# sinamalakouti/CDDMSL

Measured on AMD Instinct MI355X. Metric: images/sec (train step) VOC+Clipart RN50-C4, higher is better.
Workload: dtype bf16

## Files before the change

### __graft_entry__.py

```python
import glob
import os
import subprocess
import sys

ROOT = os.path.dirname(os.path.abspath(__file__))
CSRC = os.path.join(ROOT, "cddmsl_amd", "csrc")
LIB = os.path.join(ROOT, "cddmsl_amd", "libcddmsl_hip.so")
SIDE_LIBS = {"rpn_sparse.hip": os.path.join(ROOT, "cddmsl_amd", "libcddmsl_rpn_sparse.so")}
OBJDIR = os.path.join(ROOT, "build", "obj")
HIPCC = os.environ.get("HIPCC", "/opt/rocm/bin/hipcc")
HIPFLAGS = ["--offload-arch=gfx950", "-O3", "-fPIC", "-std=c++17", "-Wno-unused-result", "-ffp-contract=off"]


def _newer(src, dst, extra=()):
    if not os.path.exists(dst):
        return True
    t = os.path.getmtime(dst)
    return any(os.path.getmtime(s) > t for s in (src, *extra))


def build(verbose=False):
    os.makedirs(OBJDIR, exist_ok=True)
    headers = glob.glob(os.path.join(CSRC, "*.h")) + glob.glob(os.path.join(ROOT, "include", "*.h"))
    srcs = sorted(glob.glob(os.path.join(CSRC, "*.hip")))
    objs = []
    procs = []
    for s in srcs:
        o = os.path.join(OBJDIR, os.path.basename(s)[:-4] + ".o")
        objs.append(o)
        if _newer(s, o, headers):
            cmd = [HIPCC, *HIPFLAGS, "-I", os.path.join(ROOT, "include"), "-c", s, "-o", o]
            if verbose:
                print(" ".join(cmd))
            procs.append((s, subprocess.Popen(cmd)))
    for s, p in procs:
        if p.wait() != 0:
            raise RuntimeError(f"hipcc failed on {s}")
    side = {os.path.join(OBJDIR, name[:-4] + ".o"): lib for name, lib in SIDE_LIBS.items()}
    for lib, members in [(LIB, [o for o in objs if o not in side])] + [(lib, [o]) for o, lib in side.items()]:
        if not os.path.exists(lib) or any(os.path.getmtime(o) > os.path.getmtime(lib) for o in members):
            subprocess.check_call([HIPCC, "--offload-arch=gfx950", "-shared", "-fPIC", *members, "-o", lib])
    omk = os.path.join(ROOT, "oracle", "Makefile")
    if os.path.exists(omk):
        subprocess.check_call(["make", "-s", "-C", os.path.join(ROOT, "oracle")])
    if ROOT not in sys.path:
        sys.path.insert(0, ROOT)
    import cddmsl_amd
    from cddmsl_amd import _lib

    _lib.lib()
    _lib.lib_rpn_sparse()


def smoke():
    if ROOT not in sys.path:
        sys.path.insert(0, ROOT)
    import torch
    from cddmsl_amd import _lib, synthetic
    from cddmsl_amd.config import get_cfg
    from cddmsl_amd.engine import SimpleTrainer
    from cddmsl_amd.modeling import TransformerMapper, build_model
    from cddmsl_amd.solver import build_optimizer
    _lib.lib()
    assert torch.cuda.is_available(), "smoke() needs the MI355X"
    cfg = get_cfg()
    cfg.merge_from_file(os.path.join(ROOT, "configs", "VOC-Experiments", "faster_rcnn_CLIP_R_50_C4.yaml"))
    cfg.merge_from_list(["MODEL.COMPUTE_DTYPE", "f32", "MODEL.ROI_HEADS.BATCH_SIZE_PER_IMAGE", 16, "MODEL.RPN.PRE_NMS_TOPK_TRAIN", 300,
                         "MODEL.RPN.POST_NMS_TOPK_TRAIN", 100, "MODEL.DEVICE", "cuda:0"])
    sd, msd = synthetic.make_state_dict(0), synthetic.make_mapper_state_dict(1)
    model = build_model(cfg)
    model.load_state_dict(sd, strict=False)
    mapper = TransformerMapper(compute_dtype=model.compute_dtype)
    mapper.load_state_dict(msd)
    mapper.to(model.device)
    g = torch.Generator().manual_seed(3)
    model.proposal_generator.sample_generator = model.roi_heads.sample_generator = model.region_generator = g
    batch = synthetic.make_batch(1, 128, 160, num_gt=2)
    tr = SimpleTrainer(model, iter([batch]), build_optimizer(cfg, model), cfg, clipcap_model=mapper, metrics_period=0)
    tr.iter = 20000
    losses = tr.run_step()
    got = {k: float(v.detach()) for k, v in losses.items()}

    from oracle import model as om
    ocfg = om.Cfg(roi_batch_per_image=16, rpn_pre_nms_topk=300, rpn_post_nms_topk=100)
    torch.set_num_threads(min(16, os.cpu_count() or 8))
    with torch.no_grad():
        ref = om.run_step_losses(sd, msd, ocfg, batch, 20000, torch.Generator().manual_seed(3))
    for k, v in ref.items():
        assert abs(got[k] - float(v)) <= 1e-3 * abs(float(v)) + 1e-6, (k, got[k], float(v))
    print("smoke ok:", got)


if __name__ == "__main__":
    build(verbose=True)
    print("built", LIB)
```

### cddmsl_amd/_lib.py

```python
import ctypes
import os
import re

import torch

_HERE = os.path.dirname(os.path.abspath(__file__))
LIB_PATH = os.path.join(_HERE, "libcddmsl_hip.so")
HEADER_PATH = os.path.join(os.path.dirname(_HERE), "include", "cddmsl_hip.h")
RPN_SPARSE_LIB_PATH = os.path.join(_HERE, "libcddmsl_rpn_sparse.so")
RPN_SPARSE_HEADER_PATH = os.path.join(os.path.dirname(_HERE), "include", "cddmsl_rpn_sparse.h")

_lib = None
_lib_rpn_sparse = None


class HipLibraryError(RuntimeError):
    pass


_BY_VALUE = {"int": ctypes.c_int, "long": ctypes.c_long, "float": ctypes.c_float}


def _statements(header_text):
    text = re.sub(r"/\*.*?\*/", " ", header_text, flags=re.S)
    text = re.sub(r"^\s*#.*$", " ", text, flags=re.M)
    text = re.sub(r'extern\s+"C"\s*\{|^\s*\}\s*$', " ", text, flags=re.M)
    return [" ".join(s.split()) for s in text.split(";") if s.strip()]


def header_signatures(header_text):
    sigs = {}
    for st in _statements(header_text):
        if "(" not in st:
            continue
        m = re.fullmatch(r"(.*?)\b(cddmsl_\w+) ?\((.*)\)", st)
        if m is None:
            raise HipLibraryError(f"include/cddmsl_hip.h: cannot parse the declaration `{st}`")
        ret, name, params = m.group(1).strip(), m.group(2), m.group(3).strip()
        if ret != "int":
            raise HipLibraryError(f"include/cddmsl_hip.h: {name} returns `{ret}`; every entry point returns int")
        argtypes = []
        for p in ([] if params == "void" else params.split(",")):
            if "*" in p:
                argtypes.append(ctypes.c_void_p)
                continue
            words = [w for w in p.split() if w != "const"]
            if len(words) != 2 or words[0] not in _BY_VALUE:
                raise HipLibraryError(f"include/cddmsl_hip.h: {name}: parameter `{p.strip()}` is neither a pointer nor a "
                                      "by-value int / long / float")
            argtypes.append(_BY_VALUE[words[0]])
        sigs[name] = argtypes
    return sigs


def header_struct(header_text, name):
    m = re.search(r"typedef struct %s \{(.*?)\} %s;" % (name, name), re.sub(r"/\*.*?\*/", " ", header_text, flags=re.S), flags=re.S)
    if m is None:
        raise HipLibraryError(f"include/cddmsl_hip.h: no struct {name}")
    fields = []
    for st in (s.split() for s in m.group(1).split(";") if s.strip()):
        if st[0] not in ("int", "long"):
            raise HipLibraryError(f"include/cddmsl_hip.h: struct {name}: unknown member type in `{' '.join(st)}`")
        fields += [(w.strip(","), _BY_VALUE[st[0]]) for w in st[1:]]
    return fields


def _load(lib_path, header_path):
    if not os.path.exists(lib_path):
        raise HipLibraryError(
            f"{lib_path} is missing: run `python -c 'import __graft_entry__ as g; g.build()'` "
            "(hipcc --offload-arch=gfx950).  cddmsl_amd has no fallback path."
        )
    L = ctypes.CDLL(lib_path)
    with open(header_path) as f:
        sigs = header_signatures(f.read())
    for name, argtypes in sigs.items():
        fn = getattr(L, name, None)
        if fn is None:
            raise HipLibraryError(f"{lib_path} is stale: it does not export {name}, which include/{os.path.basename(header_path)} declares; rebuild it")
        fn.restype, fn.argtypes = ctypes.c_int, argtypes
    return L


def lib():
    global _lib
    if _lib is None:
        _lib = _load(LIB_PATH, HEADER_PATH)
    return _lib


def lib_rpn_sparse():
    global _lib_rpn_sparse
    if _lib_rpn_sparse is None:
        _lib_rpn_sparse = _load(RPN_SPARSE_LIB_PATH, RPN_SPARSE_HEADER_PATH)
    return _lib_rpn_sparse


def stream_ptr():
    return ctypes.c_void_p(torch._C._cuda_getCurrentRawStream(torch.cuda.current_device()))


def to_device_async(cpu_tensor, device):
    if torch.device(device).type == "cpu":
        return cpu_tensor
    if cpu_tensor.numel() == 0:
        return torch.empty(cpu_tensor.shape, dtype=cpu_tensor.dtype, device=device)
    return cpu_tensor.pin_memory().to(device, non_blocking=True)


def ptr(t):
    if t is None:
        return ctypes.c_void_p(0)
    return ctypes.c_void_p(t.data_ptr())


def check(status, what):
    if status != 0:
        raise HipLibraryError(f"{what} failed with status {status}")


def require_cuda(*tensors):
    for t in tensors:
        if t is not None and not t.is_cuda:
            raise HipLibraryError(
                "cddmsl_amd ops run only on the MI355X HIP path; got a CPU tensor "
                "(the CPU restatement lives in oracle/ and is test infrastructure only)"
            )


class Readback:

    def __init__(self, t):
        if t.is_cuda:
            self.host = torch.empty(t.shape, dtype=t.dtype, pin_memory=True)
            self.host.copy_(t, non_blocking=True)
            self.ev = torch.cuda.Event()
            self.ev.record()
        else:
            self.host, self.ev = t, None

    def get(self):
        if self.ev is not None:
            self.ev.synchronize()
        return self.host
```

### cddmsl_amd/csrc/conv_wgrad.hip

```cpp
#include "gemm_common.h"

namespace {

template <typename T> struct TrFrag;
template <> struct TrFrag<__bf16> {
  __device__ static __forceinline__ u32x4 read(const u32x4* base, int mrow0, int col0, int lane) {
    int g = lane >> 4, li = lane & 15, q = li >> 2, pp = li & 3;
    int hh = g >> 1;
    int col = col0 + 16 * (g & 1) + 4 * pp;
    const char* b = (const char*)base;
    const char* a0 = b + (long)(mrow0 + 8 * hh + q) * (WROW * 16) + col * 2;
    const char* a1 = a0 + 4 * (WROW * 16);
    i16x4 v0 = __builtin_amdgcn_ds_read_tr16_b64_v4i16((__attribute__((address_space(3))) i16x4*)a0);
    i16x4 v1 = __builtin_amdgcn_ds_read_tr16_b64_v4i16((__attribute__((address_space(3))) i16x4*)a1);
    u32x2 p0 = __builtin_bit_cast(u32x2, v0), p1 = __builtin_bit_cast(u32x2, v1);
    u32x4 r = {p0[0], p0[1], p1[0], p1[1]};
    return r;
  }
  static constexpr int MSTEP = 16;
};
template <> struct TrFrag<float> {
  __device__ static __forceinline__ u32x4 read(const u32x4* base, int mrow0, int col0, int lane) {
    int r = lane & 31, hh = lane >> 5;
    const char* b = (const char*)base;
// ... 83 lines not shown
    for (int ms = 0; ms < WM; ms += TrFrag<T>::MSTEP) {
      u32x4 fa[NT], fb[NT];
#pragma unroll
      for (int i = 0; i < NT; ++i) {
        fa[i] = TrFrag<T>::read(lds[0], ms, wn * WT + i * 32, lane);
        fb[i] = TrFrag<T>::read(lds[1], ms, wk * WT + i * 32, lane);
      }
#pragma unroll
      for (int a = 0; a < NT; ++a)
#pragma unroll
        for (int b = 0; b < NT; ++b) Mma<T>::step(acc[a][b], fa[a], fb[b]);
    }
    __syncthreads();
  }

  const int r = lane & 31, h = lane >> 5;
#pragma unroll
  for (int a = 0; a < NT; ++a)
#pragma unroll
    for (int b = 0; b < NT; ++b) {
      int k = k0 + wk * WT + b * 32 + r;
      if (k >= p.K) continue;
#pragma unroll
      for (int g = 0; g < 16; ++g) {
        int n = n0 + wn * WT + a * 32 + (g & 3) + 8 * (g >> 2) + 4 * h;
        if (n >= p.Cout) continue;
        float v = acc[a][b][g] * (p.scale ? p.scale[n] : 1.f);
        atomicAdd(p.dw + (long)n * p.K + k, v);
      }
    }
}


template <typename T> struct TrFragS;
template <> struct TrFragS<__bf16> {
  struct Off { int o0, o1; };
  __device__ static __forceinline__ Off prep(int col0, int lane) {
    int g = lane >> 4, li = lane & 15, q = li >> 2, pp = li & 3;
    int hh = g >> 1;
    int ch = ((col0 + 16 * (g & 1)) >> 3) + (pp >> 1);
    int r0 = 8 * hh + q, r1 = r0 + 4;
    Off o;
    o.o0 = r0 * 256 + 16 * (ch ^ fsw(r0)) + 8 * (pp & 1);
    o.o1 = r1 * 256 + 16 * (ch ^ fsw(r1)) + 8 * (pp & 1);
    return o;
  }
  __device__ static __forceinline__ u32x4 read(const u32x4* base, int ms, const Off& o) {
    const unsigned a = (unsigned)(size_t)(const __attribute__((address_space(3))) char*)((const char*)base) + ms * 256;
    u32x2 p0, p1;
    asm volatile("ds_read_b64_tr_b16 %0, %1" : "=v"(p0) : "v"(a + o.o0));
    asm volatile("ds_read_b64_tr_b16 %0, %1" : "=v"(p1) : "v"(a + o.o1));
    u32x4 r = {p0[0], p0[1], p1[0], p1[1]};
    return r;
  }
  static constexpr int MSTEP = 16;
};
template <> struct TrFragS<float> {
  struct Off { int o[4]; };
  __device__ static __forceinline__ Off prep(int col0, int lane) {
    int r = lane & 31, hh = lane >> 5;
    int byte = (col0 + r) * 4;
    Off o;
#pragma unroll
    for (int j = 0; j < 4; ++j) {
      int row = 4 * hh + j;
      o.o[j] = row * 256 + (byte & 15) + 16 * (byte >> 4);
    }
    return o;
  }
  __device__ static __forceinline__ u32x4 read(const u32x4* base, int ms, const Off& o) {
    const char* b = (const char*)base;
    u32x4 v;
#pragma unroll
    for (int j = 0; j < 4; ++j) {
      int off = o.o[j] + ms * 256;
      int row = off >> 8, ch = (off >> 4) & 15;
      v[j] = *(const unsigned int*)(b + (off & ~0xf0) + 16 * (ch ^ fsw(row)));
    }
    return v;
  }
  static constexpr int MSTEP = 8;
};

template <typename T>
__global__ __launch_bounds__(256, 2) void k_conv_wgrad_dma(WgradArgs p) {
  constexpr int ES = Mma<T>::ES;
  constexpr int COLS = 256 / ES;
  __shared__ __attribute__((aligned(16))) u32x4 lds[2][2][WM * 16];
  const int t = threadIdx.x, lane = t & 63, wv = t >> 6;
  p.x += (long)blockIdx.y * p.bx; p.dy += (long)blockIdx.y * p.bd;
  char* outp = (char*)p.dw + (long)blockIdx.y * p.bo;
  const int wvu = __builtin_amdgcn_readfirstlane(t >> 6);
  const int ntn = (p.Cout + COLS - 1) / COLS, ntk = (p.K + COLS - 1) / COLS;
  int bid = xcd_remap(blockIdx.x, gridDim.x);
  const int tile_k = bid % ntk; bid /= ntk;
  const int tile_n = bid % ntn; bid /= ntn;
  const int split = bid;
  const int n0 = tile_n * COLS, k0 = tile_k * COLS;
  const int mt0 = split * p.mtiles_per_split;
  const int total_mt = (p.M + WM - 1) / WM;
  const int mt1 = min(mt0 + p.mtiles_per_split, total_mt);

  const int cc = t & 15, rb = t >> 4;
  const int cl = cc ^ fsw(rb);
  const int kc = k0 * ES / 16 + cl;
  const bool vk = kc < p.Kc;
  const int pp = vk ? kc / p.cpp : 0, coff = vk ? kc - pp * p.cpp : 0;
  const int ky = pp / p.KW, kx = pp - ky * p.KW;
  const int nc = n0 * ES / 16 + cl;
  const bool vn = nc < p.ncc;
  const bool taps = !(p.KH == 1 && p.KW == 1);
  const char* zp = (const char*)g_zero_page;

  int m[4];
  const char* pd[4];
  const char* px[4];
#pragma unroll
  for (int i = 0; i < 4; ++i) {
    m[i] = mt0 * WM + rb + 16 * i;
    pd[i] = p.dy + ((long)m[i] * p.ldd) * ES + (long)nc * 16;
    px[i] = p.x + (((long)m[i] + (long)(ky - p.pad) * p.Wi + (kx - p.pad)) * p.xrs) * 16 + (long)coff * 16;
  }
  const long dstep = (long)WM * p.ldd * ES, xstep = (long)WM * p.xrs * 16;

  auto stage = [&](int buf) {
#pragma unroll
    for (int i = 0; i < 4; ++i) {
      bool vmm = m[i] < p.M;
      glds16((vmm && vn) ? pd[i] : zp, &lds[buf][0][(4 * wvu + 16 * i) * 16]);
    }
#pragma unroll
    for (int i = 0; i < 4; ++i) {
      bool ok = (m[i] < p.M) & vk;
      if (taps) {
        unsigned mm = min((unsigned)m[i], (unsigned)(p.M - 1));
        unsigned tq = fdiv(mm, p.dWo);
        unsigned ox = mm - tq * p.Wo;
        unsigned oy = tq - fdiv(tq, p.dHo) * p.Ho;
        ok = ok & ((unsigned)((int)oy - p.pad + ky) < (unsigned)p.Hi) & ((unsigned)((int)ox - p.pad + kx) < (unsigned)p.Wi);
      }
      glds16(ok ? px[i] : zp, &lds[buf][1][(4 * wvu + 16 * i) * 16]);
    }
#pragma unroll
    for (int i = 0; i < 4; ++i) { m[i] += WM; pd[i] += dstep; px[i] += xstep; }
  };

  constexpr int WT = COLS / 2;
  constexpr int NT = WT / 32;
  const int wn = wv >> 1, wk = wv & 1;
  f32x16 acc[NT][NT];
#pragma unroll
  for (int a = 0; a < NT; ++a)
#pragma unroll
    for (int b = 0; b < NT; ++b)
#pragma unroll
      for (int r = 0; r < 16; ++r) acc[a][b][r] = 0.f;

  typename TrFragS<T>::Off offa[NT], offb[NT];
#pragma unroll
  for (int i = 0; i < NT; ++i) {
    offa[i] = TrFragS<T>::prep(wn * WT + i * 32, lane);
    offb[i] = TrFragS<T>::prep(wk * WT + i * 32, lane);
  }

  if (mt0 < mt1) stage(0);
  for (int mt = mt0; mt < mt1; ++mt) {
    const int cur = (mt - mt0) & 1;
    if (mt + 1 < mt1) {
      stage(cur ^ 1);
      asm volatile("s_waitcnt vmcnt(8)" ::: "memory");
    } else {
      asm volatile("s_waitcnt vmcnt(0)" ::: "memory");
    }
    __builtin_amdgcn_s_barrier();
#pragma unroll
    for (int ms = 0; ms < WM; ms += TrFragS<T>::MSTEP) {
      u32x4 fa[NT], fb[NT];
#pragma unroll
      for (int i = 0; i < NT; ++i) {
        fa[i] = TrFragS<T>::read(lds[cur][0], ms, offa[i]);
        fb[i] = TrFragS<T>::read(lds[cur][1], ms, offb[i]);
      }
      asm volatile("s_waitcnt lgkmcnt(0)" ::: "memory");
      __builtin_amdgcn_sched_barrier(0);
#pragma unroll
      for (int a = 0; a < NT; ++a)
#pragma unroll
        for (int b = 0; b < NT; ++b) Mma<T>::step(acc[a][b], fa[a], fb[b]);
    }
    asm volatile("s_waitcnt lgkmcnt(0)" ::: "memory");
    __builtin_amdgcn_s_barrier();
  }

  const int r = lane & 31, h = lane >> 5;
  if (p.ws) {
    f32x4* dst = (f32x4*)p.ws + ((long)(split * ntn + tile_n) * ntk + tile_k) * (4 * NT * NT * 4 * 64) + (wv * NT * NT * 4) * 64 + lane;
#pragma unroll
    for (int a = 0; a < NT; ++a)
#pragma unroll
      for (int b = 0; b < NT; ++b)
#pragma unroll
        for (int g4 = 0; g4 < 4; ++g4) {
          const f32x4 v = {acc[a][b][4 * g4], acc[a][b][4 * g4 + 1], acc[a][b][4 * g4 + 2], acc[a][b][4 * g4 + 3]};
          dst[((a * NT + b) * 4 + g4) * 64] = v;
        }
    return;
  }
#pragma unroll
  for (int a = 0; a < NT; ++a)
#pragma unroll
    for (int b = 0; b < NT; ++b) {
      int k = k0 + wk * WT + b * 32 + r;
      if (k >= p.K) continue;
#pragma unroll
      for (int g = 0; g < 16; ++g) {
        int n = n0 + wn * WT + a * 32 + (g & 3) + 8 * (g >> 2) + 4 * h;
        if (n >= p.Cout) continue;
        float v = acc[a][b][g] * (p.scale ? p.scale[n] : 1.f);
        long o = (long)n * p.ldo + k;
        if (p.direct == 0) atomicAdd((float*)outp + o, v);
        else if (p.direct == 1) ((float*)outp)[o] = v;
        else Mma<T>::store(outp + o * ES, v);
      }
    }
}

template <typename T>
__global__ __launch_bounds__(256, 2) void k_gemm_tn_stream(WgradArgs p, int nbatch, int bpb) {
  constexpr int ES = Mma<T>::ES;
  constexpr int COLS = 256 / ES;
  __shared__ __attribute__((aligned(16))) u32x4 lds[2][2][WM * 16];
  const int t = threadIdx.x, lane = t & 63, wv = t >> 6;
  const int wvu = __builtin_amdgcn_readfirstlane(t >> 6);
  const int ntk = (p.K + COLS - 1) / COLS;
  const int tile_k = blockIdx.x % ntk, tile_n = blockIdx.x / ntk;
  const int n0 = tile_n * COLS, k0 = tile_k * COLS;
  const int b0 = blockIdx.y * bpb, nb = min(bpb, nbatch - b0);
  const int nmt = (p.M + WM - 1) / WM;
  const int nit = nb * nmt;

  const int cc = t & 15, rb = t >> 4;
  const int cl = cc ^ fsw(rb);
  const int kc = k0 * ES / 16 + cl, nc = n0 * ES / 16 + cl;
  const bool vk = kc < p.Kc, vn = nc < p.ncc;
  const char* zp = (const char*)g_zero_page;
  int sb = 0, smt = 0;
  auto stage = [&](int buf) {
    const char* db = p.dy + (long)(b0 + sb) * p.bd + (long)nc * 16;
    const char* xb = p.x + (long)(b0 + sb) * p.bx + (long)kc * 16;
#pragma unroll
    for (int i = 0; i < 4; ++i) {
      const int m = smt * WM + rb + 16 * i;
// ... 185 lines not shown
    const unsigned x0 = sbase + xoff[0], x1 = sbase + xoff[1];
    CDDMSL_TRS(fb[0], x0, x1, 0) CDDMSL_TRS(fb[1], x0, x1, 4096) CDDMSL_TRS(fb[2], x0, x1, 8192) CDDMSL_TRS(fb[3], x0, x1, 12288)
#pragma unroll
    for (int a = 0; a < NTN; ++a) {
      const unsigned a0 = sbase + aoff[a][0], a1 = sbase + aoff[a][1];
      CDDMSL_TRS(fa[a][0], a0, a1, 0) CDDMSL_TRS(fa[a][1], a0, a1, 2048) CDDMSL_TRS(fa[a][2], a0, a1, 4096) CDDMSL_TRS(fa[a][3], a0, a1, 6144)
    }
#undef CDDMSL_TRS
    if (NTN == 1) asm volatile("s_waitcnt lgkmcnt(0)" : "+v"(fb[0]), "+v"(fb[1]), "+v"(fb[2]), "+v"(fb[3]), "+v"(fa[0][0]), "+v"(fa[0][1]),
                               "+v"(fa[0][2]), "+v"(fa[0][3]) :: "memory");
    else asm volatile("s_waitcnt lgkmcnt(0)" : "+v"(fb[0]), "+v"(fb[1]), "+v"(fb[2]), "+v"(fb[3]), "+v"(fa[0][0]), "+v"(fa[0][1]), "+v"(fa[0][2]),
                      "+v"(fa[0][3]), "+v"(fa[NTN - 1][0]), "+v"(fa[NTN - 1][1]), "+v"(fa[NTN - 1][2]), "+v"(fa[NTN - 1][3]) :: "memory");
    __builtin_amdgcn_sched_barrier(0);
#pragma unroll
    for (int ms = 0; ms < 4; ++ms)
#pragma unroll
      for (int a = 0; a < NTN; ++a) Mma<__bf16>::step(acc[a], fa[a][ms], fb[ms]);
    __builtin_amdgcn_s_barrier();
    char* outp = (char*)p.dw + (long)(b0 + it) * p.bo;
    const int k = k0 + wvu * 32 + r;
    if (MODE == 3) {
      if (kind == 2) asm volatile("s_waitcnt vmcnt(6)" : "+v"(g0v), "+v"(mbv) :: "memory");
      else asm volatile("s_waitcnt vmcnt(0)" : "+v"(g0v), "+v"(mbv) :: "memory");
      const unsigned a00 = __builtin_bit_cast(unsigned, acc[0][0]);
      const float t0 = __builtin_bit_cast(float, __builtin_amdgcn_permlane32_swap(a00, a00, false, false)[0]) + g0v;
      const float base = t0 * (1.0f / (float)(P > 0 ? P : 1));
      const unsigned mlo = mbv[0], mhi = mbv[1];
#pragma unroll
      for (int a = 0; a < NTN; ++a)
#pragma unroll
        for (int g = 0; g < 16; ++g) {
          const int n0 = a * 32 + (g & 3) + 8 * (g >> 2);
          const bool exists = a * 4 + (g >> 2) < NG;
          const bool lo_ok = n0 >= 1 && n0 <= P, hi_ok = n0 + 4 >= 1 && n0 + 4 <= P;
          if (exists) {
            const int n = n0 + 4 * h;
            const float v = acc[a][g];
            gacc[a][g] += (n == 0) ? t0 : v;
            if (lo_ok || hi_ok) {
              if (h ? hi_ok : lo_ok) {
                const unsigned word = (n - 1) < 32 ? mlo : mhi;
                const bool keep = (word >> ((n - 1) & 31)) & 1u;
                Mma<__bf16>::store(outp + ((long)(n - 1) * p.ldo + k) * 2, keep ? v + base : 0.f);
              }
            }
          }
          acc[a][g] = 0.f;
        }
      return;
    }
#pragma unroll
    for (int a = 0; a < NTN; ++a)
#pragma unroll
      for (int g = 0; g < 16; ++g) {
        if (a * 4 + (g >> 2) < NG) {
          const int n = a * 32 + (g & 3) + 8 * (g >> 2) + 4 * h;
          const float v = acc[a][g];
          const long o = (long)n * p.ldo + k;
          if (MODE == 0) atomicAdd((float*)outp + o, v);
          else if (MODE == 1) ((float*)outp)[o] = v;
          else Mma<__bf16>::store(outp + o * 2, v);
        }
        acc[a][g] = 0.f;
      }
  };
  {
    int it = 0;
    for (; it + 2 < nit; ++it) item(it, std::integral_constant<int, 2>{});
    if (it + 1 < nit) { item(it, std::integral_constant<int, 1>{}); ++it; }
    if (it < nit) item(it, std::integral_constant<int, 0>{});
  }
  if (MODE == 3 && p.gpos) {
    const int k = k0 + wvu * 32 + r;
#pragma unroll
    for (int a = 0; a < NTN; ++a)
#pragma unroll
      for (int g = 0; g < 16; ++g) {
        const int n = a * 32 + (g & 3) + 8 * (g >> 2) + 4 * h;
        if (a * 4 + (g >> 2) < NG && n <= P) atomicAdd(p.gpos + (long)n * p.K + k, gacc[a][g]);
      }
  }
}

__global__ __launch_bounds__(512) void k_wgrad256(WgradArgs p) {
  __shared__ __attribute__((aligned(16))) u32x4 lds[2 * 2 * 2 * 64 * 16];
  const int t = threadIdx.x, lane = t & 63;
#ifdef CDDMSL_TILE_STAMPS
  const unsigned long long ts_entry = __builtin_amdgcn_s_memrealtime();
  unsigned long long ts_loop = ts_entry;
#endif
  p.x += (long)blockIdx.y * p.bx; p.dy += (long)blockIdx.y * p.bd;
  char* outp = (char*)p.dw + (long)blockIdx.y * p.bo;
  const int wvu = __builtin_amdgcn_readfirstlane(t >> 6);
  const int wn = wvu >> 2, wk = wvu & 3;
  const int ntn = p.Cout >> 8, ntk = p.K >> 8;
  int bid = xcd_remap(blockIdx.x, gridDim.x);
  const int tile_k = bid % ntk; bid /= ntk;
  const int tile_n = bid % ntn; bid /= ntn;
  const int n0 = tile_n * 256, k0 = tile_k * 256;
  const int mt0 = bid * p.mtiles_per_split;
  const int nmt = min(p.mtiles_per_split, (p.M + WM - 1) / WM - mt0);
  const bool taps = !(p.KH == 1 && p.KW == 1);

  const int rb = t >> 4, cl = (t & 15) ^ fsw(rb);
  const int gd = (cl >> 3) * 16 + (cl & 7);
  const int gx = (cl >> 2) * 8 + (cl & 3);
  const int kc = (k0 >> 3) + gx;
  const int pp = kc / p.cpp, coff = kc - pp * p.cpp;
  const int ky = pp / p.KW, kx = pp - ky * p.KW;
  unsigned vd[2], vx[2];
#pragma unroll
  for (int i = 0; i < 2; ++i) {
    vd[i] = (unsigned)((i * 32 + rb) * p.ldd * 2 + gd * 16);
    vx[i] = (unsigned)((((i * 32 + rb) + ky * p.Wi + kx) * p.xrs + coff) * 16);
  }
  const __amdgpu_buffer_rsrc_t rd = __builtin_amdgcn_make_buffer_rsrc((void*)(p.dy + ((long)mt0 * WM * p.ldd + n0) * 2), 0, 0x80000000u, 0x00020000);
  const __amdgpu_buffer_rsrc_t rx = __builtin_amdgcn_make_buffer_rsrc((void*)(p.x + ((long)mt0 * WM - p.pad * p.Wi - p.pad) * p.xrs * 16), 0, 0x80000000u, 0x00020000);
  const unsigned dstep = (unsigned)(WM * p.ldd * 2), xstep = (unsigned)(WM * p.xrs * 16);
  const int mrow = mt0 * WM + rb;

  char* const L = (char*)lds;
  auto stageD = [&](auto H, int buf, int T) {
    constexpr int h = decltype(H)::value;
    char* dst = L + (buf << 16) + (h << 14) + wvu * 1024;
#pragma unroll
    for (int i = 0; i < 2; ++i) {
      const unsigned inv = (mrow + T * WM + i * 32 < p.M) ? 0u : 0x80000000u;
      __builtin_amdgcn_raw_ptr_buffer_load_lds(rd, (__attribute__((address_space(3))) void*)(dst + i * 8192 - h * 128), 16,
                                               (int)(vd[i] | inv), (int)(T * dstep), h * 128, 0);
    }
  };
  unsigned xinv[2];
  auto validX = [&](int T) {
#pragma unroll
    for (int i = 0; i < 2; ++i) {
      const int m = mrow + T * WM + i * 32;
      bool ok = m < p.M;
      if (taps) {
        const unsigned mm = min((unsigned)m, (unsigned)(p.M - 1));
        const unsigned tq = fdiv(mm, p.dWo);
        const unsigned ox = mm - tq * p.Wo;
        const unsigned oy = tq - fdiv(tq, p.dHo) * p.Ho;
        ok = ok & ((unsigned)((int)oy - p.pad + ky) < (unsigned)p.Hi) & ((unsigned)((int)ox - p.pad + kx) < (unsigned)p.Wi);
      }
      xinv[i] = ok ? 0u : 0x80000000u;
    }
  };
  auto stageX = [&](auto J, int buf, int T) {
    constexpr int j = decltype(J)::value;
    char* dst = L + (buf << 16) + (1 << 15) + (j << 14) + wvu * 1024;
#pragma unroll
    for (int i = 0; i < 2; ++i)
      __builtin_amdgcn_raw_ptr_buffer_load_lds(rx, (__attribute__((address_space(3))) void*)(dst + i * 8192 - j * 64), 16,
                                               (int)(vx[i] | xinv[i]), (int)(T * xstep), j * 64, 0);
  };
  using I0 = std::integral_constant<int, 0>;
  using I1 = std::integral_constant<int, 1>;

  f32x16 acc[4][2];
#pragma unroll
  for (int a = 0; a < 4; ++a)
#pragma unroll
    for (int b = 0; b < 2; ++b)
#pragma unroll
      for (int r = 0; r < 16; ++r) acc[a][b][r] = 0.f;

  const unsigned lbase = (unsigned)(size_t)(__attribute__((address_space(3))) char*)L;
  unsigned adA[2][2], adB[2];
  {
#pragma unroll
    for (int a = 0; a < 2; ++a) {
      const TrFragS<__bf16>::Off o = TrFragS<__bf16>::prep(wn * 64 + a * 32, lane);
      adA[a][0] = lbase + o.o0; adA[a][1] = lbase + o.o1;
    }
    const TrFragS<__bf16>::Off o = TrFragS<__bf16>::prep(wk * 32, lane);
    adB[0] = lbase + (1u << 15) + o.o0; adB[1] = lbase + (1u << 15) + o.o1;
  }
  u32x4 fa0[2][4], fa1[2][4], fb0[4], fb1[4];
#define CDDMSL_TR2(DST, A0, A1, IMM)                                                             \
  { u32x2 q0_, q1_;                                                                              \
    asm volatile("ds_read_b64_tr_b16 %0, %1 offset:%2" : "=v"(q0_) : "v"(A0), "i"(IMM));         \
    asm volatile("ds_read_b64_tr_b16 %0, %1 offset:%2" : "=v"(q1_) : "v"(A1), "i"(IMM));         \
    DST = u32x4{q0_[0], q0_[1], q1_[0], q1_[1]}; }
#define CDDMSL_READ_A(HALF, FA)                                                                  \
  _Pragma("unroll") for (int a = 0; a < 2; ++a) {                                                \
    CDDMSL_TR2(FA[a][0], adA[a][0], adA[a][1], ((HALF) << 14) + 0 * 4096)                        \
    CDDMSL_TR2(FA[a][1], adA[a][0], adA[a][1], ((HALF) << 14) + 1 * 4096)                        \
    CDDMSL_TR2(FA[a][2], adA[a][0], adA[a][1], ((HALF) << 14) + 2 * 4096)                        \
    CDDMSL_TR2(FA[a][3], adA[a][0], adA[a][1], ((HALF) << 14) + 3 * 4096) }
#define CDDMSL_READ_B(HALF, FB)                                                                  \
  CDDMSL_TR2(FB[0], adB[0], adB[1], ((HALF) << 14) + 0 * 4096)                                   \
  CDDMSL_TR2(FB[1], adB[0], adB[1], ((HALF) << 14) + 1 * 4096)                                   \
  CDDMSL_TR2(FB[2], adB[0], adB[1], ((HALF) << 14) + 2 * 4096)                                   \
  CDDMSL_TR2(FB[3], adB[0], adB[1], ((HALF) << 14) + 3 * 4096)
#define CDDMSL_FLIP_A() { adA[0][0] ^= 1u << 16; adA[0][1] ^= 1u << 16; adA[1][0] ^= 1u << 16; adA[1][1] ^= 1u << 16; }
#define CDDMSL_FLIP_B() { adB[0] ^= 1u << 16; adB[1] ^= 1u << 16; }
#define CDDMSL_MMA_QUAD(I, J, FA, FB)                                               \
  _Pragma("unroll") for (int ms = 0; ms < 4; ++ms) {                                \
    Mma<__bf16>::step(acc[2 * (I)][J], FA[0][ms], FB[ms]);                          \
    Mma<__bf16>::step(acc[2 * (I) + 1][J], FA[1][ms], FB[ms]);                      \
  }
#define CDDMSL_WAIT4(F) asm volatile("s_waitcnt lgkmcnt(0)" : "+v"(F[0]), "+v"(F[1]), "+v"(F[2]), "+v"(F[3]) :: "memory");
#define CDDMSL_WAIT8(F) asm volatile("s_waitcnt lgkmcnt(0)" : "+v"(F[0][0]), "+v"(F[0][1]), "+v"(F[0][2]), "+v"(F[0][3]), \
                                     "+v"(F[1][0]), "+v"(F[1][1]), "+v"(F[1][2]), "+v"(F[1][3]) :: "memory");
#define CDDMSL_PHASE_SYNC_IN(WAIT)                                                  \
  __builtin_amdgcn_sched_barrier(0);                                                \
  __builtin_amdgcn_s_barrier();                                                     \
  WAIT                                                                              \
  __builtin_amdgcn_sched_barrier(0);                                                \
  __builtin_amdgcn_s_setprio(1);
#define CDDMSL_PHASE_SYNC_OUT(I, J)                                                 \
  asm volatile("" : "+v"(acc[2 * (I)][J]), "+v"(acc[2 * (I) + 1][J]));              \
  __builtin_amdgcn_s_setprio(0);                                                    \
  __builtin_amdgcn_sched_barrier(0);                                                \
  __builtin_amdgcn_s_barrier();                                                     \
  __builtin_amdgcn_sched_barrier(0);

  if (nmt > 0) {
    validX(0);
    stageD(I0{}, 0, 0); stageD(I1{}, 0, 0); stageX(I0{}, 0, 0); stageX(I1{}, 0, 0);
    if (nmt > 1) {
      validX(1);
      stageD(I0{}, 1, 1); stageX(I0{}, 1, 1); stageX(I1{}, 1, 1);
      asm volatile("s_waitcnt vmcnt(6)" ::: "memory");
    } else {
      asm volatile("s_waitcnt vmcnt(0)" ::: "memory");
    }
    __builtin_amdgcn_s_barrier();
    __builtin_amdgcn_sched_barrier(0);
    CDDMSL_READ_A(0, fa0)
    CDDMSL_WAIT8(fa0)
    if (wn == 1) __builtin_amdgcn_s_barrier();
    __builtin_amdgcn_sched_barrier(0);
// ... 201 lines not shown
      const unsigned a0 = adA[0] + ro, a1 = adA[1] + ro, b0 = adB[0] + ro, b1 = adB[1] + ro;
      CDDMSL_TR8x4(fa[0], a0)
      mma(IS{}, I2{}, I0{});
      CDDMSL_TR8x4(fa[1], a1)
      mma(IS{}, I2{}, I1{});
      CDDMSL_TR8x4(fb[N][0], b0)
      mma(IS{}, I3{}, I0{});
      CDDMSL_TR8x4(fb[N][1], b1)
      mma(IS{}, I3{}, I1{});
    }
  };
  if (nmt > 0) {
    stage(0);
    if (nmt > 1) stage(1);
    if (nmt > 2) stage(2);
    if (nmt > 2) asm volatile("s_waitcnt vmcnt(8)" ::: "memory");
    else if (nmt > 1) asm volatile("s_waitcnt vmcnt(4)" ::: "memory");
    else asm volatile("s_waitcnt vmcnt(0)" ::: "memory");
    __builtin_amdgcn_sched_barrier(0);
    __builtin_amdgcn_s_barrier();
    __builtin_amdgcn_sched_barrier(0);
    CDDMSL_TR8x4(fa[0], adA[0]) CDDMSL_TR8x4(fa[1], adA[1]) CDDMSL_TR8x4(fb[0][0], adB[0]) CDDMSL_TR8x4(fb[0][1], adB[1])
    for (int kt = 0; kt < nmt; kt += 2) {
      body(kt, I0{});
      body(kt + 1, I1{});
    }
  }
#undef CDDMSL_TR8x4
#undef CDDMSL_F8_WAIT_TOP
#undef CDDMSL_F8_WAIT_MID
#undef CDDMSL_TR8

  const int r = lane & 31, h = lane >> 5;
  if (p.ws) {
    store_frags((f32x4*)p.ws + ((long)(bid * ntn + tile_n) * ntk + tile_k) * (8 * 32 * 64) + (wvu * 32) * 64 + lane, acc);
  } else
#pragma unroll
  for (int a = 0; a < 4; ++a)
#pragma unroll
    for (int b = 0; b < 2; ++b) {
      const int k = k0 + wk * 64 + b * 32 + r;
#pragma unroll
      for (int g = 0; g < 16; ++g) {
        const int n = n0 + wn * 128 + a * 32 + (g & 3) + 8 * (g >> 2) + 4 * h;
        atomicAdd(p.dw + (long)n * p.ldo + k, acc[a][b][g] * (p.scale ? p.scale[n] : 1.f));
      }
    }
}

}

template <int WAVES, int FR>
__global__ __launch_bounds__(256) void k_wgrad_reduce(const f32x4* ws, float* dw, const float* scale, int ntn, int ntk, int splits, int Cout, int K, int ldo) {
  constexpr int SLOTS = WAVES * FR * 64;
  constexpr int TN = WAVES == 8 ? 256 : 128;
  const int tile = blockIdx.x / (SLOTS / 256), q = (blockIdx.x % (SLOTS / 256)) * 256 + threadIdx.x;
  const int tile_k = tile % ntk, tile_n = tile / ntk;
  const long ntiles = (long)ntn * ntk;
  const f32x4* src = ws + (long)tile * SLOTS + q;
  f32x4 sum = {0.f, 0.f, 0.f, 0.f};
  int s = 0;
  for (; s + 4 <= splits; s += 4) {
    const f32x4 a = src[(s + 0) * ntiles * SLOTS], b = src[(s + 1) * ntiles * SLOTS], c = src[(s + 2) * ntiles * SLOTS], d = src[(s + 3) * ntiles * SLOTS];
    sum += (a + b) + (c + d);
  }
  for (; s < splits; ++s) sum += src[s * ntiles * SLOTS];
  const int wv = q / (FR * 64), j = (q / 64) % FR, lane = q & 63, r = lane & 31, h = lane >> 5, g4 = j & 3;
  int a, b, wn, wk;
  if (WAVES == 8) { a = j >> 3; b = (j >> 2) & 1; wn = wv >> 2; wk = wv & 3; }
  else { a = j >> 3; b = (j >> 2) & 1; wn = wv >> 1; wk = wv & 1; }
  const int n = tile_n * TN + wn * (WAVES == 8 ? 128 : 64) + a * 32 + 8 * g4 + 4 * h;
  const int k = tile_k * TN + wk * 64 + b * 32 + r;
  if (k >= K) return;
#pragma unroll
  for (int e = 0; e < 4; ++e)
    if (n + e < Cout) dw[(long)(n + e) * ldo + k] += sum[e] * (scale ? scale[n + e] : 1.f);
}

static bool use_workspace(long blocks, long tile_floats, void* ws, long ws_bytes) {
  if (env_int("CDDMSL_WGRAD_WS", 1) == 0) return false;
  return ws != nullptr && blocks * tile_floats * 4 <= ws_bytes;
}

template <int WAVES, int FR>
static void launch_wgrad_split(void (*kernel)(WgradArgs), WgradArgs& a, const Plan& p, hipStream_t st, void* wsp, long ws_bytes) {
  constexpr int TN = WAVES == 8 ? 256 : 128, SLOTS = WAVES * FR * 64;
  const int ntn = (a.Cout + TN - 1) / TN, ntk = (a.K + TN - 1) / TN;
  const bool ws = p.splits > 1 && use_workspace((long)p.gx, SLOTS * 4, wsp, ws_bytes);
  if (ws) a.ws = (float*)wsp;
  hipLaunchKernelGGL(kernel, dim3(p.gx), dim3(WAVES * 64), 0, st, a);
  if (ws) hipLaunchKernelGGL((k_wgrad_reduce<WAVES, FR>), dim3((unsigned)(ntn * ntk * (SLOTS / 256))), dim3(256), 0, st, (const f32x4*)wsp, a.dw, a.scale,
                             ntn, ntk, p.splits, a.Cout, a.K, a.ldo);
}

void launch_wgrad(WgradArgs& a, const Plan& p, Operand op, hipStream_t st, void* ws, long ws_bytes) {
  switch (p.kernel) {
    case 12: launch_wgrad_split<8, 32>(k_wgrad256_f8, a, p, st, ws, ws_bytes); break;
    case 6: launch_wgrad_split<8, 32>(k_wgrad256, a, p, st, ws, ws_bytes); break;
    case 5:
      if (op == OP_BF16) launch_wgrad_split<4, 16>(k_conv_wgrad_dma<__bf16>, a, p, st, ws, ws_bytes);
      else hipLaunchKernelGGL(k_conv_wgrad_dma<float>, dim3(p.gx), dim3(256), 0, st, a);
      break;
    default:
      if (op == OP_BF16) hipLaunchKernelGGL(k_conv_wgrad<__bf16>, dim3(p.gx), dim3(256), 0, st, a);
      else hipLaunchKernelGGL(k_conv_wgrad<float>, dim3(p.gx), dim3(256), 0, st, a);
  }
}

void launch_gemm_tn(const WgradArgs& p, Operand op, const Plan& pl, int batch, int mode, hipStream_t st) {
  const dim3 grid(pl.gx, pl.gy);
  if (pl.kernel == 9) {
#define CDDMSL_TNS(NG)                                                                                              \
  case NG:                                                                                                          \
    if (mode == 0) hipLaunchKernelGGL((k_gemm_tn_small<NG, 0>), grid, dim3(256), 0, st, p, batch, pl.bpb);      \
    else if (mode == 1) hipLaunchKernelGGL((k_gemm_tn_small<NG, 1>), grid, dim3(256), 0, st, p, batch, pl.bpb); \
    else hipLaunchKernelGGL((k_gemm_tn_small<NG, 2>), grid, dim3(256), 0, st, p, batch, pl.bpb);                \
    break;
    switch (p.Cout / 8) { CDDMSL_TNS(1) CDDMSL_TNS(2) CDDMSL_TNS(3) CDDMSL_TNS(4) CDDMSL_TNS(5) CDDMSL_TNS(6) CDDMSL_TNS(7) CDDMSL_TNS(8) }
#undef CDDMSL_TNS
  } else if (pl.kernel == 7) {
    if (op == OP_BF16) hipLaunchKernelGGL(k_gemm_tn_stream<__bf16>, grid, dim3(256), 0, st, p, batch, pl.bpb);
    else hipLaunchKernelGGL(k_gemm_tn_stream<float>, grid, dim3(256), 0, st, p, batch, pl.bpb);
  } else {
    if (op == OP_BF16) hipLaunchKernelGGL(k_conv_wgrad_dma<__bf16>, grid, dim3(256), 0, st, p);
    else hipLaunchKernelGGL(k_conv_wgrad_dma<float>, grid, dim3(256), 0, st, p);
  }
}

void launch_attnpool_dx(const WgradArgs& p, unsigned gx, unsigned gy, int nbatch, int bpb, hipStream_t st) {
  hipLaunchKernelGGL((k_gemm_tn_small<7, 3, 49>), dim3(gx, gy), dim3(256), 0, st, p, nbatch, bpb);
}
```

### cddmsl_amd/csrc/gemm_common.h

```cpp
#pragma once
#include "common.h"
#include <cstdlib>

namespace {

constexpr int BM = 128, BN = 128, KCH = 8;

struct FastDiv {
  unsigned mul, shr, d;
};
static inline FastDiv make_fastdiv(unsigned d) {
  FastDiv f;
  f.d = d;
  unsigned s = 0;
  while ((1ull << s) < d) ++s;
  f.shr = s;
  f.mul = (unsigned)(((1ull << 32) * ((1ull << s) - d)) / d + 1);
  return f;
}
__device__ __forceinline__ unsigned fdiv(unsigned n, const FastDiv& f) { return (__umulhi(n, f.mul) + n) >> f.shr; }

template <typename T> __device__ __forceinline__ float affine(float v, float sc, float bi) {
  return sizeof(T) <= 2 ? __builtin_fmaf(v, sc, bi) : v * sc + bi;
}
// ... 31 lines not shown
  FastDiv dWp = {}, dHp = {};
  int nt_out = 1;
#ifdef CDDMSL_TILE_STAMPS
  unsigned long long* tstamps = nullptr;
#endif
};

template <typename T> struct Mma;
template <> struct Mma<__bf16> {
  static constexpr int ES = 2;
  __device__ static __forceinline__ void step(f32x16& acc, const u32x4& a, const u32x4& b) {
    acc = __builtin_amdgcn_mfma_f32_32x32x16_bf16(__builtin_bit_cast(bf16x8, a), __builtin_bit_cast(bf16x8, b), acc, 0, 0, 0);
  }
  __device__ static __forceinline__ float load(const char* p) { return bf2f(*(const unsigned short*)p); }
  __device__ static __forceinline__ void store(char* p, float v) { *(unsigned short*)p = f2bf(v); }
};
template <> struct Mma<float> {
  static constexpr int ES = 4;
  __device__ static __forceinline__ void step(f32x16& acc, const u32x4& a, const u32x4& b) {
    const f32x4 fa = __builtin_bit_cast(f32x4, a), fb = __builtin_bit_cast(f32x4, b);
    acc = __builtin_amdgcn_mfma_f32_32x32x2f32(fa[0], fb[0], acc, 0, 0, 0);
    acc = __builtin_amdgcn_mfma_f32_32x32x2f32(fa[1], fb[1], acc, 0, 0, 0);
    acc = __builtin_amdgcn_mfma_f32_32x32x2f32(fa[2], fb[2], acc, 0, 0, 0);
    acc = __builtin_amdgcn_mfma_f32_32x32x2f32(fa[3], fb[3], acc, 0, 0, 0);
  }
  __device__ static __forceinline__ float load(const char* p) { return *(const float*)p; }
  __device__ static __forceinline__ void store(char* p, float v) { *(float*)p = v; }
};
typedef __attribute__((ext_vector_type(8))) int i32x8;

__device__ __forceinline__ int xcd_remap(int bid, int nblk) {
  const int q = nblk >> 3, rem = nblk & 7, x = bid & 7, j = bid >> 3;
  return (x < rem ? x * (q + 1) : rem * (q + 1) + (x - rem) * q) + j;
}

template <typename T> __device__ __forceinline__ u32x4 avg4(const u32x4& a, const u32x4& b, const u32x4& c, const u32x4& d);
template <> __device__ __forceinline__ u32x4 avg4<float>(const u32x4& a, const u32x4& b, const u32x4& c, const u32x4& d) {
  const f32x4 fa = __builtin_bit_cast(f32x4, a), fb = __builtin_bit_cast(f32x4, b);
  const f32x4 fc = __builtin_bit_cast(f32x4, c), fd = __builtin_bit_cast(f32x4, d);
  f32x4 r = ((fa + fb) + (fc + fd)) * 0.25f;
  return __builtin_bit_cast(u32x4, r);
}
template <> __device__ __forceinline__ u32x4 avg4<__bf16>(const u32x4& a, const u32x4& b, const u32x4& c, const u32x4& d) {
  u32x4 r;
#pragma unroll
  for (int j = 0; j < 4; ++j) {
    float lo = (bf2f(a[j] & 0xffff) + bf2f(b[j] & 0xffff)) + (bf2f(c[j] & 0xffff) + bf2f(d[j] & 0xffff));
    float hi = (bf2f(a[j] >> 16) + bf2f(b[j] >> 16)) + (bf2f(c[j] >> 16) + bf2f(d[j] >> 16));
    r[j] = pack2bf(lo * 0.25f, hi * 0.25f);
  }
  return r;
}

__device__ __attribute__((aligned(16))) unsigned int g_zero_page[4] = {0u, 0u, 0u, 0u};

__device__ __forceinline__ void glds16(const void* g, void* l) {
  __builtin_amdgcn_global_load_lds((const __attribute__((address_space(1))) void*)g,
                                   (__attribute__((address_space(3))) void*)l, 16, 0, 0);
}

struct WgradArgs {
  const char* x;
  const char* dy;
  float* dw;
  const float* scale;
  int Nimg, Hi, Wi, Cin, Ho, Wo, Cout, KH, KW, stride, pad, ldd, pool;
  int M, Kc, cpp, K, ncc;
  int mtiles_per_split;
  FastDiv dWo, dHo;
  int xrs;
  int ldo;
  int direct;
  long bx, bd, bo;
  const float* g0 = nullptr;
  const unsigned long long* mbits = nullptr;
  float* gpos = nullptr;
  float* ws = nullptr;
#ifdef CDDMSL_TILE_STAMPS
  unsigned long long* tstamps = nullptr;
#endif
};

constexpr int WM = 64;
constexpr int WROW = 16 + 4;

__device__ __forceinline__ int fsw(int row) { return ((row & 3) << 2) | ((row >> 2) & 3); }

__device__ __forceinline__ void store_frags(f32x4* dst, const f32x16 (&acc)[4][2]) {
#pragma unroll
  for (int a = 0; a < 4; ++a)
#pragma unroll
    for (int b = 0; b < 2; ++b)
#pragma unroll
      for (int g4 = 0; g4 < 4; ++g4) {
        const f32x4 v = {acc[a][b][4 * g4], acc[a][b][4 * g4 + 1], acc[a][b][4 * g4 + 2], acc[a][b][4 * g4 + 3]};
        dst[((a * 2 + b) * 4 + g4) * 64] = v;
      }
}

static long env_int(const char* name, long dflt, bool* set = nullptr) {
  const char* e = getenv(name);
  if (set) *set = e != nullptr;
  return e ? atol(e) : dflt;
}

enum Operand { OP_BF16 = 0, OP_F32 = 1, OP_FP8 = 2 };
static int elem_size(Operand op) { return op == OP_BF16 ? 2 : op == OP_F32 ? 4 : 1; }

struct Plan {
  int kernel;
  unsigned gx, gy;
  int splits;
  int mtiles_per_split;
  int bpb;
};

static int persistent_blocks_raw() {
  static int ncu = -1;
  if (ncu < 0) {
    int dev = 0, n = 0;
    if (hipGetDevice(&dev) != hipSuccess || hipDeviceGetAttribute(&n, hipDeviceAttributeMultiprocessorCount, dev) != hipSuccess) n = 0;
    ncu = (n / 8) * 8;
  }
  return ncu;
}

}

extern "C" {
__attribute__((visibility("hidden"))) void launch_fwd_tile128(const ConvArgs& a, const Plan& p, Operand op, hipStream_t st);
__attribute__((visibility("hidden"))) void launch_fwd_tile256(const ConvArgs& a, const Plan& p, Operand op, hipStream_t st, void* ws, long ws_bytes);
__attribute__((visibility("hidden"))) void launch_wgrad(WgradArgs& a, const Plan& p, Operand op, hipStream_t st, void* ws, long ws_bytes);
__attribute__((visibility("hidden"))) void launch_gemm_tn(const WgradArgs& p, Operand op, const Plan& pl, int batch, int mode, hipStream_t st);
__attribute__((visibility("hidden"))) void launch_attnpool_dx(const WgradArgs& p, unsigned gx, unsigned gy, int nbatch, int bpb, hipStream_t st);
__attribute__((visibility("hidden"))) bool record_kernel(int id);
}
```

### cddmsl_amd/csrc/gemm_conv.hip

```cpp
#include "gemm_common.h"

namespace {

template <typename T>
__device__ __forceinline__ void weight_prep_body(const float* w, const float* scale, char* wf, char* wd, int Cout, int KH, int KW, int Cin,
                                                 long first, long stride) {
  __shared__ float tile[32][33];
  const int taps = KH * KW, nit = (Cin + 31) / 32, nct = (Cout + 31) / 32;
  const long ntiles = (long)nct * taps * nit;
  const int tx = threadIdx.x & 31, ty = threadIdx.x >> 5;
  constexpr int ES = Mma<T>::ES;
  for (long tl = first; tl < ntiles; tl += stride) {
    const int it = (int)(tl % nit); const long q = tl / nit;
    const int tap = (int)(q % taps), ct = (int)(q / taps);
    const int ky = tap / KW, kx = tap % KW;
    __syncthreads();
#pragma unroll
    for (int r = 0; r < 4; ++r) {
      const int co = ct * 32 + ty + 8 * r, ci = it * 32 + tx;
      float v = 0.f;
      if (co < Cout && ci < Cin) {
        const long i = ((long)co * taps + tap) * Cin + ci;
        v = w[i];
        if (wf) Mma<T>::store(wf + i * ES, v);
        if (scale) v *= scale[co];
      }
      tile[ty + 8 * r][tx] = v;
    }
    __syncthreads();
    if (wd) {
#pragma unroll
      for (int r = 0; r < 4; ++r) {
        const int ci = it * 32 + ty + 8 * r, co = ct * 32 + tx;
        if (ci < Cin && co < Cout) {
          const long j = (((long)ci * KH + (KH - 1 - ky)) * KW + (KW - 1 - kx)) * Cout + co;
          Mma<T>::store(wd + j * ES, tile[tx][ty + 8 * r]);
        }
      }
    }
  }
}
template <typename T>
__global__ __launch_bounds__(256) void k_weight_prep(const float* w, const float* scale, char* wf, char* wd, int Cout, int KH, int KW, int Cin) {
  weight_prep_body<T>(w, scale, wf, wd, Cout, KH, KW, Cin, (long)blockIdx.x, (long)gridDim.x);
}
template <typename T>
__global__ __launch_bounds__(256) void k_weight_prep_multi(const long long* table) {
  const long long* e = table + 8 * (long)blockIdx.y;
  weight_prep_body<T>((const float*)e[0], (const float*)e[1], (char*)e[2], (char*)e[3], (int)e[4], (int)e[5], (int)e[6], (int)e[7],
                      (long)blockIdx.x, (long)gridDim.x);
}

static thread_local int g_last_kernel = 0;
static thread_local int g_plan_only = 0;


static bool gemm256_legal(const ConvArgs& a) {
  const bool vec_ok = (a.ldy % 8 == 0) && (!a.residual || a.ldr % 8 == 0) && (!a.relu_mask || a.ldm % 8 == 0);
  if (a.pool || (a.cpp & 7) || (a.Cout & 255) || !vec_ok || a.KH * a.KW > 31) return false;
  if (2 * a.pad > a.KH - 1 || 2 * a.pad > a.KW - 1) return false;
  return true;
}

static bool use_gemm256(const ConvArgs& a, int batch) {
  const long mode = env_int("CDDMSL_GEMM256", 1);
  if (mode == 0) return false;
  if (!gemm256_legal(a)) return false;
  if (mode == 2) return true;
  const long tiles = (long)((a.M + 255) / 256) * (a.Cout / 256) * batch;
  return tiles >= 160;
}

static bool fwd2_legal(const ConvArgs& a) {
  const bool vec_ok = (a.ldy % 8 == 0) && (!a.residual || a.ldr % 8 == 0) && (!a.relu_mask || a.ldm % 8 == 0);
  if (a.pool || a.res_pool || (a.cpp & 3) || (a.Cout & 127) || !vec_ok || a.KH * a.KW > 31) return false;
  if (2 * a.pad > a.KH - 1 || 2 * a.pad > a.KW - 1) return false;
  return true;
}
static bool use_fwd2(const ConvArgs& a, int batch) {
  const long mode = env_int("CDDMSL_FWD2", 1);
  if (mode == 0 || !fwd2_legal(a)) return false;
  if (mode == 2) return true;
  if (use_gemm256(a, batch) || batch != 1) return false;
// ... 60 lines not shown
  a.x = (const char*)x; a.w = (const char*)w; a.y = (char*)y; a.scale = scale; a.bias = bias;
  a.residual = (const char*)residual; a.relu_mask = (const char*)relu_mask;
  a.Nimg = Nimg; a.Hi = Hi; a.Wi = Wi; a.Cin = Cin; a.Cout = Cout; a.KH = KH; a.KW = KW; a.stride = stride; a.pad = pad;
  if (pool) { a.Ho = Hi / 2; a.Wo = Wi / 2; }
  else { a.Ho = (Hi + 2 * pad - KH) / stride + 1; a.Wo = (Wi + 2 * pad - KW) / stride + 1; }
  if (a.Ho <= 0 || a.Wo <= 0) return CDDMSL_ERR_ARG;
  if ((out_f32 & 2) && (!(out_f32 & 1) || !residual || relu_mask || pool)) return CDDMSL_ERR_ARG;
  a.ldy = ldy; a.ldr = ldr; a.ldm = ldm; a.relu = relu; a.out_f32 = out_f32 & 1; a.pool = pool;
  a.res_f32 = (op == OP_BF16 && (out_f32 & 2)) ? 1 : 0;
  a.res_pool = (out_f32 & 4) ? 1 : 0;
  if (a.res_pool && (!residual || (out_f32 & 2) || pool || KH != 1 || KW != 1 || pad != 0 || (long)Nimg * (a.Ho / 2) * (a.Wo / 2) * ldr * es >= (1L << 31) ||
                     (Cout & 7) || (ldy & 7) || (ldr & 7) || (relu_mask && (ldm & 7)))) return CDDMSL_ERR_ARG;
  if (a.res_f32 && ((Cout & 7) || (ldy & 7) || (ldr & 7))) return CDDMSL_ERR_ARG;
  long M = (long)Nimg * a.Ho * a.Wo;
  if (M > 0x7fffff00L) return CDDMSL_ERR_ARG;
  a.M = (int)M; a.cpp = Cin * es / 16; a.Kc = KH * KW * a.cpp;
  a.dWo = make_fastdiv((unsigned)a.Wo); a.dHo = make_fastdiv((unsigned)a.Ho);
  a.dcpp = make_fastdiv((unsigned)a.cpp); a.dKW = make_fastdiv((unsigned)KW);
  a.xrs = a.cpp; a.wrs = a.Kc; a.bx = a.bw = a.by = 0;
#ifdef CDDMSL_TILE_STAMPS
  a.tstamps = g_tile_stamps;
#endif
  if (a.M == 0) return CDDMSL_OK;
  a.nt_out = nt_out_for((long)a.M * Cout * 2);
  if (y8) {
    if (op == OP_F32 || (out_f32 & 1) || ldy != Cout) return CDDMSL_ERR_ARG;
    a.y8 = (char*)y8; a.q8 = q8; a.amax8 = (unsigned*)amax8;
  }
  return CDDMSL_OK;
}

static int conv_fwd_any(Operand op, const void* x, const void* w, void* y, const float* scale, const float* bias,
                        const void* residual, const void* relu_mask, int Nimg, int Hi, int Wi, int Cin,
                        int Cout, int KH, int KW, int stride, int pad, int pool, int ldy, int ldr, int ldm,
                        int relu, int out_f32, void* y8, const float* q8, float* amax8, void* stream) {
  ConvArgs a;
  const int st = fill_conv(a, op, x, w, y, scale, bias, residual, relu_mask, Nimg, Hi, Wi, Cin, Cout, KH, KW, stride, pad, pool, ldy, ldr, ldm,
                           relu, out_f32, y8, q8, amax8);
  if (st != CDDMSL_OK || a.M == 0) return st;
  return run_fwd(a, op, plan_fwd(a, op, 1), stream);
}

extern "C" int cddmsl_conv_fwd(const void* x, const void* w, void* y, const float* scale, const float* bias,
                               const void* residual, const void* relu_mask, int Nimg, int Hi, int Wi, int Cin,
                               int Cout, int KH, int KW, int stride, int pad, int pool, int ldy, int ldr, int ldm,
                               int relu, int out_f32, int dtype, void* stream) {
  if (dtype != 0 && dtype != 1) return CDDMSL_ERR_ARG;
  return conv_fwd_any((Operand)dtype, x, w, y, scale, bias, residual, relu_mask, Nimg, Hi, Wi, Cin, Cout, KH, KW, stride, pad, pool, ldy, ldr, ldm,
                      relu, out_f32, nullptr, nullptr, nullptr, stream);
}

extern "C" int cddmsl_conv3x3_pool_fwd(const void* x, const void* w, void* y, const float* scale, const float* bias, const void* relu_mask,
                                       int Nimg, int Hi, int Wi, int Cin, int Cout, int stride, int dtype, void* stream) {
  if (dtype != 0 || Cin != 32 || Cout != 64 || stride != 1 || relu_mask || !scale || !bias || Hi < 2 || Wi < 2) return CDDMSL_ERR_ARG;
  ConvArgs a;
  const int st = fill_conv(a, OP_BF16, x, w, y, scale, bias, nullptr, nullptr, Nimg, Hi, Wi, Cin, Cout, 3, 3, 1, 1, 0, Cout, 0, 0, 1, 0,
                           nullptr, nullptr, nullptr);
  if (st != CDDMSL_OK || a.M == 0) return st;
  if ((long)Nimg * Hi * Wi * Cin * 2 >= 0x7ffff000L || (long)Nimg * (a.Ho / 2) * (a.Wo / 2) * Cout * 2 >= 0x7fffffffL) return CDDMSL_ERR_ARG;
  a.pool_out = 1;
  a.dWp = make_fastdiv((unsigned)(a.Wo / 2)); a.dHp = make_fastdiv((unsigned)(a.Ho / 2));
  const Plan pl = plan_fwd(a, OP_BF16, 1);
  if (pl.kernel != 8) return CDDMSL_ERR_ARG;
  return run_fwd(a, OP_BF16, pl, stream);
}

extern "C" int cddmsl_conv_fwd_q8(const void* x, const void* w, void* y, const float* scale, const float* bias,
                                  const void* residual, const void* relu_mask, int Nimg, int Hi, int Wi, int Cin,
                                  int Cout, int KH, int KW, int stride, int pad, int relu, void* y8, const float* q8, float* amax8,
                                  void* stream) {
  if (!y8) return CDDMSL_ERR_ARG;
  return conv_fwd_any(OP_BF16, x, w, y, scale, bias, residual, relu_mask, Nimg, Hi, Wi, Cin, Cout, KH, KW, stride, pad, 0, Cout, Cout, Cout,
                      relu, 0, y8, q8, amax8, stream);
}

extern "C" int cddmsl_conv_fwd_fp8(const void* x, const void* w, void* y, const float* scale, const float* bias,
                                   const void* residual, const void* relu_mask, int Nimg, int Hi, int Wi, int Cin, int Cout, int KH,
                                   int KW, int pad, int relu, int out_f32, void* y8, const float* q8, float* amax8, void* stream) {
  if (Cin % 128 != 0 || (out_f32 & ~1)) return CDDMSL_ERR_ARG;
  return conv_fwd_any(OP_FP8, x, w, y, scale, bias, residual, relu_mask, Nimg, Hi, Wi, Cin, Cout, KH, KW, 1, pad, 0, Cout, Cout, Cout,
                      relu, out_f32, y8, q8, amax8, stream);
}

static bool wgrad256_ok(const WgradArgs& a, int batch) {
  const long mode = env_int("CDDMSL_GEMM256", 1);
  if (mode == 0) return false;
  if ((a.Cout & 255) || (a.K & 255) || (a.cpp & 7) || (a.ldd & 7)) return false;
  if (mode == 2) return true;
  return (long)(a.Cout / 256) * (a.K / 256) * batch * ((a.M + WM - 1) / WM) >= env_int("CDDMSL_WGRAD256_MIN", 4000);
}
static bool wgrad256_span_ok(int mtiles_per_split, int Wi, long row_bytes) {
  return ((long)mtiles_per_split * WM + WM + 2L * Wi + 2) * row_bytes + (1L << 20) < (1L << 31);
}

static int even_split(int total_mt, long* splits) {
  const int mps = (int)((total_mt + *splits - 1) / *splits);
  *splits = (total_mt + mps - 1) / mps;
  return mps;
}

static long split_512_rounds(long tiles, int total_mt, bool taps) {
  bool forced;
  const long target = env_int("CDDMSL_WGRAD_BLOCKS", taps ? 1024 : 512, &forced);
  const long maxs = (total_mt + 7) / 8;
  long splits = 1;
  const long r0 = (target + 511) / 512;
  double best = -1.0;
  for (long r = r0; r <= r0 + 1; ++r) {
    long c = (512 * r) / tiles;
    if (c < 1) c = 1;
    if (c > maxs) c = maxs;
    long real = c;
    even_split(total_mt, &real);
    const long blocks = tiles * real, rounds = (blocks + 511) / 512;
    const double eff = (double)blocks / (512.0 * rounds);
    if (eff > best + 0.03) { best = eff; splits = c; }
    if (c == maxs) break;
  }
  if (forced) { splits = (target + tiles - 1) / tiles; if (splits > maxs) splits = maxs; }
  return splits < 1 ? 1 : splits;
}

static long split_256_rounds(long tiles, int total_mt) {
  const long maxs = (total_mt + 15) / 16;
  long sp = 1;
  double best = -1.0;
  for (int r = 1; r <= 6; ++r) {
    long c = (256L * r) / tiles;
    if (c < 1) continue;
    if (c > maxs) c = maxs;
    const long blocks = tiles * c, rounds = (blocks + 255) / 256;
    const double eff = (double)blocks / (256.0 * rounds);
    if (eff > best + 0.02) { best = eff; sp = c; }
    if (c == maxs) break;
  }
  return sp;
}

static Plan plan_wgrad(const WgradArgs& a, Operand op, int batch) {
  const int es = elem_size(op), total_mt = (a.M + WM - 1) / WM;
  const long tiles256 = (long)(a.Cout / 256) * (a.K / 256);
  const long row_bytes = (long)a.ldd * es > a.xrs * 16L ? (long)a.ldd * es : a.xrs * 16L;
  if (op == OP_FP8) {
    long sp = split_256_rounds(tiles256, total_mt);
    const int mps = even_split(total_mt, &sp);
    if (!wgrad256_span_ok(mps, a.Wi, row_bytes)) return {};
    return {12, (unsigned)(tiles256 * sp), 1, (int)sp, mps};
  }
  const int cols = 256 / es;
  const long tiles = (long)((a.Cout + cols - 1) / cols) * ((a.K + cols - 1) / cols);
  long splits = split_512_rounds(tiles, total_mt, !(a.KH == 1 && a.KW == 1));
  const int mps = even_split(total_mt, &splits);
  if (tiles * splits > 0x7fffffffL) return {};
  const bool same = !a.pool && a.stride == 1 && a.Ho == a.Hi && a.Wo == a.Wi;
  if (same && op == OP_BF16 && wgrad256_ok(a, batch)) {
    bool forced;
    const long want = env_int("CDDMSL_WGRAD256_BLOCKS", 0, &forced);
    const long maxs = (total_mt + 15) / 16;
    long sp = forced ? (want + tiles256 - 1) / tiles256 : split_256_rounds(tiles256, total_mt);
    if (sp > maxs) sp = maxs;
    if (sp < 1) sp = 1;
    const int mps256 = even_split(total_mt, &sp);
    if (wgrad256_span_ok(mps256, a.Wi, row_bytes)) return {6, (unsigned)(tiles256 * sp), 1, (int)sp, mps256};
  }
  return {same ? 5 : 4, (unsigned)(tiles * splits), 1, (int)splits, mps};
}

extern "C" int cddmsl_set_workspace(void* ptr, long bytes) {
  if (bytes < 0 || (ptr == nullptr && bytes != 0) || ((size_t)ptr & 15)) return CDDMSL_ERR_ARG;
  g_ws = ptr; g_ws_bytes = bytes;
  return CDDMSL_OK;
}

static int run_wgrad(WgradArgs& a, Operand op, const Plan& p, void* stream) {
  if (p.kernel == 0) return CDDMSL_ERR_ARG;
  g_last_kernel = p.kernel;
  if (g_plan_only) return CDDMSL_OK;
  a.mtiles_per_split = p.mtiles_per_split;
  launch_wgrad(a, p, op, (hipStream_t)stream, g_ws, g_ws_bytes);
  return launch_status();
}

static int fill_wgrad(WgradArgs& a, Operand op, const void* x, const void* dy, float* dw, const float* scale, int Nimg, int Hi,
                      int Wi, int Cin, int Cout, int KH, int KW, int stride, int pad, int pool, int ldd) {
  const int es = elem_size(op);
  if (Nimg < 0 || Hi <= 0 || Wi <= 0 || Cin <= 0 || Cout <= 0 || KH <= 0 || KW <= 0 || stride <= 0) return CDDMSL_ERR_ARG;
  if ((Cin * es) % 16 != 0 || (Cout * es) % 16 != 0 || (ldd * es) % 16 != 0) return CDDMSL_ERR_ARG;
  if (pool && (KH != 1 || KW != 1 || pad != 0 || stride != 1)) return CDDMSL_ERR_ARG;
  a.x = (const char*)x; a.dy = (const char*)dy; a.dw = dw; a.scale = scale;
  a.Nimg = Nimg; a.Hi = Hi; a.Wi = Wi; a.Cin = Cin; a.Cout = Cout; a.KH = KH; a.KW = KW; a.stride = stride; a.pad = pad;
  a.ldd = ldd; a.pool = pool;
  if (pool) { a.Ho = Hi / 2; a.Wo = Wi / 2; }
  else { a.Ho = (Hi + 2 * pad - KH) / stride + 1; a.Wo = (Wi + 2 * pad - KW) / stride + 1; }
  if (a.Ho <= 0 || a.Wo <= 0) return CDDMSL_ERR_ARG;
  long M = (long)Nimg * a.Ho * a.Wo;
  if (M > 0x7fffff00L) return CDDMSL_ERR_ARG;
  a.M = (int)M; a.cpp = Cin * es / 16; a.Kc = KH * KW * a.cpp; a.K = KH * KW * Cin; a.ncc = Cout * es / 16;
  a.mtiles_per_split = 0;
  a.dWo = make_fastdiv((unsigned)a.Wo); a.dHo = make_fastdiv((unsigned)a.Ho);
  a.xrs = a.cpp; a.ldo = a.K; a.direct = 0; a.bx = a.bd = a.bo = 0;
#ifdef CDDMSL_TILE_STAMPS
  a.tstamps = g_tile_stamps;
#endif
  return CDDMSL_OK;
}

extern "C" int cddmsl_conv_wgrad(const void* x, const void* dy, float* dw, const float* scale, int Nimg, int Hi,
                                 int Wi, int Cin, int Cout, int KH, int KW, int stride, int pad, int pool, int ldd,
                                 int dtype, void* stream) {
  if (dtype != 0 && dtype != 1) return CDDMSL_ERR_ARG;
  WgradArgs a;
  const int st = fill_wgrad(a, (Operand)dtype, x, dy, dw, scale, Nimg, Hi, Wi, Cin, Cout, KH, KW, stride, pad, pool, ldd);
  if (st != CDDMSL_OK || a.M == 0) return st;
  return run_wgrad(a, (Operand)dtype, plan_wgrad(a, (Operand)dtype, 1), stream);
}

extern "C" int cddmsl_conv_wgrad_fp8_ok(int Cin, int Cout, int KH, int KW, int pad, int ldd) {
  return (Cin % 256 == 0 && Cout % 256 == 0 && KH == KW && (KH & 1) && 2 * pad == KH - 1 && ldd % 16 == 0) ? 1 : 0;
}
extern "C" int cddmsl_conv_wgrad_fp8(const void* x8, const void* dy8, float* dw, const float* scale, int Nimg, int Hi, int Wi, int Cin,
                                     int Cout, int KH, int KW, int pad, int ldd, void* stream) {
  if (!cddmsl_conv_wgrad_fp8_ok(Cin, Cout, KH, KW, pad, ldd) || ldd < Cout) return CDDMSL_ERR_ARG;
  WgradArgs a;
  const int st = fill_wgrad(a, OP_FP8, x8, dy8, dw, scale, Nimg, Hi, Wi, Cin, Cout, KH, KW, 1, pad, 0, ldd);
  if (st != CDDMSL_OK || a.M == 0) return st;
  return run_wgrad(a, OP_FP8, plan_wgrad(a, OP_FP8, 1), stream);
}

extern "C" int cddmsl_gemm_nt_batched(const void* a, const void* w, void* c, const float* bias, int M, int N, int K, int lda,
                                      int ldb, int ldc, int batch, long sa, long sw, long sc, int out_f32, int dtype, void* stream) {
  int es = dtype == 0 ? 2 : 4;
  if (dtype != 0 && dtype != 1) return CDDMSL_ERR_ARG;
  if (M < 0 || N <= 0 || K <= 0 || batch < 0 || batch > 65535) return CDDMSL_ERR_ARG;
  if ((K * es) % 16 || (lda * es) % 16 || (ldb * es) % 16 || (sa * es) % 16 || (sw * es) % 16) return CDDMSL_ERR_ARG;
  if (M == 0 || batch == 0) return CDDMSL_OK;
  const Operand op = (Operand)dtype;
  ConvArgs p;
  const int st = fill_conv(p, op, a, w, c, nullptr, bias, nullptr, nullptr, 1, 1, M, K, N, 1, 1, 1, 0, 0, ldc, 0, 0, 0, out_f32 ? 1 : 0,
                           nullptr, nullptr, nullptr);
  if (st != CDDMSL_OK) return st;
  p.xrs = lda * es / 16; p.wrs = ldb * es / 16;
  p.bx = sa * es; p.bw = sw * es; p.by = sc * (out_f32 ? 4 : es);
  p.nt_out = 1;
  return run_fwd(p, op, plan_fwd(p, op, batch), stream);
}

static unsigned tn_small_grid(long kt, long batch, int* bpb) {
  long b = (kt * batch + 4095) / 4096;
  if (b < 8) b = 8;
  if (b > batch) b = batch;
  *bpb = (int)b;
  return (unsigned)((batch + b - 1) / b);
}

static Plan plan_gemm_tn(const WgradArgs& p, Operand op, int batch, int mode) {
  const int cols = 256 / elem_size(op), M = p.M, N = p.Cout, K = p.K;
  const long tiles = (long)((N + cols - 1) / cols) * ((K + cols - 1) / cols);
  const int total_mt = (M + WM - 1) / WM;
  if (op == OP_BF16 && total_mt == 1 && N <= 64 && batch >= 64 && K % 128 == 0 && N % 8 == 0) {
    Plan p = {9, (unsigned)(K / 128), 0};
    p.gy = tn_small_grid(K / 128, batch, &p.bpb);
    return p;
  }
  if (total_mt <= 4 && batch >= 64) {
    long bpb = (tiles * batch + 4095) / 4096, minb = (8 + total_mt - 1) / total_mt;
    if (bpb < minb) bpb = minb;
    if (bpb > batch) bpb = batch;
    return {7, (unsigned)tiles, (unsigned)((batch + bpb - 1) / bpb), 0, 0, (int)bpb};
  }
  long splits = 1;
  if (mode == 0) {
    const long want = (2048 + tiles * batch - 1) / (tiles * batch), maxs = (total_mt + 7) / 8;
    splits = want < 1 ? 1 : (want > maxs ? maxs : want);
    if (splits < 1) splits = 1;
  }
  const int mps = even_split(total_mt, &splits);
  if (tiles * splits > 0x7fffffffL) return {};
  return {5, (unsigned)(tiles * splits), (unsigned)batch, (int)splits, mps};
}

extern "C" int cddmsl_gemm_tn_batched(const void* a, const void* b, void* out, int M, int N, int K, int lda, int ldb, int ldo,
                                      int batch, long sa, long sb, long so, int mode, int dtype, void* stream) {
  int es = dtype == 0 ? 2 : 4;
  if (dtype != 0 && dtype != 1) return CDDMSL_ERR_ARG;
  if (M <= 0 || N <= 0 || K <= 0 || batch <= 0 || batch > 65535 || mode < 0 || mode > 2) return CDDMSL_ERR_ARG;
  if ((K * es) % 16 || (N * es) % 16 || (lda * es) % 16 || (ldb * es) % 16 || (sa * es) % 16 || (sb * es) % 16) return CDDMSL_ERR_ARG;
  const Operand op = (Operand)dtype;
// ... 51 lines not shown
```

### cddmsl_amd/engine.py

```python
import os
import time

import torch
import torch.distributed as dist

from .modeling.clipcap import TransformerMapper
from .hip import same_layout
from .solver import build_optimizer


def get_world_size():
    return dist.get_world_size() if dist.is_available() and dist.is_initialized() else 1


def get_rank():
    return dist.get_rank() if dist.is_available() and dist.is_initialized() else 0


def init_distributed(backend=None):
    ws = int(os.environ.get("WORLD_SIZE", "1"))
    if ws > 1 and not dist.is_initialized():
        os.environ.setdefault("HSA_ENABLE_IPC_MODE_LEGACY", "0")
        if torch.cuda.is_available():
            torch.cuda.set_device(0 if os.environ.get("CDDMSL_SHARE_GPU") else int(os.environ.get("LOCAL_RANK", "0")))
# ... 121 lines not shown

    def all_reduce_mean(self):
        from . import layers
        layers._TOUCH_HOOK[0] = None
        ws = get_world_size()
        if ws == 1:
            return
        if self._counting is not None:
            self._expected[self._sig] = self._counting
            self._counting = None
        if self._left is not None and any(v != 0 for v in self._left.values()):
            late = [bi for bi in self._launched if any(self._left.get(q, 0) != 0 for q in self._bucket_params[bi])]
            if late:
                raise RuntimeError("GradBuckets: fewer gradient writes than expected reached buckets already reduced")
        self._ready = []
        for bi in range(len(self.buckets)):
            if bi not in self._launched:
                self._launch(bi)
        for h, bi in self._handles:
            if self.compression is None or not self.buckets[bi].is_cuda:
                h.wait()
                if self.compression is not None:
                    self.buckets[bi].copy_(self._wire[bi])
            else:
                with torch.cuda.stream(self._comm_stream):
                    h.wait()
                    self.buckets[bi].copy_(self._wire[bi])
        if self._comm_stream is not None:
            torch.cuda.current_stream().wait_stream(self._comm_stream)
        self._handles, self._left, self._open = [], None, None
        self._launched, self._ready = set(), []


class SimpleTrainer:
    def __init__(self, model, data_loader, optimizer, cfg, clipcap_model=None, metrics_period=20):
        model.train()
        self.model, self.cfg = model, cfg
        if clipcap_model is None:
            clipcap_model = TransformerMapper(1024, 768, 40, 40, 8, compute_dtype=model.compute_dtype)
            path = cfg.MODEL.get("VISION_TO_LANG_PATH", "")
            if path and os.path.exists(path):
                sd = torch.load(path, map_location="cpu", weights_only=True)
                clipcap_model.load_state_dict({k[len("clip_project."):]: v for k, v in sd.items() if k.startswith("clip_project.")})
            clipcap_model.to(model.device)
        self.clipcap_model = clipcap_model.eval()
        for p in self.clipcap_model.parameters():
            p.requires_grad = False
        self.data_loader = data_loader
        self._data_loader_iter = iter(data_loader)
        self.optimizer = optimizer
        self.buckets = GradBuckets(optimizer.params)
        self.iter = 0
        self.burn_in = 10000
        self.metrics_period = metrics_period
        self.storage = {}
        self.share_source_pass = os.environ.get("CDDMSL_SHARE_SOURCE_PASS", "1") != "0"
        self.fuse_consistency = os.environ.get("CDDMSL_FUSE_CONSISTENCY", "1") != "0"

    def compute_losses(self, data):
        kd = self.cfg.MODEL.KD_REGULRAZIATION
        if hasattr(self.model, "share_source_pass"):
            self.model.share_source_pass = self.share_source_pass and self.iter > self.burn_in
        loss_dict = self.model(data)
        loss = {}
        if self.iter > self.burn_in and self.fuse_consistency and hasattr(self.model, "forward_consistency"):
            loss.update(self.model(data, clipcap_model=self.clipcap_model, branch="caption_consistency_both", KD_regularization=kd))
        elif self.iter > self.burn_in:
            loss.update(self.model(data, clipcap_model=self.clipcap_model, branch="caption_consistency", KD_regularization=kd))
            loss["cont_region_loss"] = self.model(data, clipcap_model=self.clipcap_model,
                                                  branch="caption_consistency_regionLevel", KD_regularization=kd)
        else:
            cc = self.model(data, clipcap_model=self.clipcap_model, branch="caption_consistency", KD_regularization=False)
            for k in cc:
                loss[k] = cc[k] * 0.0
        loss_dict.update(loss)
        return loss_dict

    def run_step(self):
        assert self.model.training, "[SimpleTrainer] model was changed to eval mode!"
        start = time.perf_counter()
        data = next(self._data_loader_iter)
        data_time = time.perf_counter() - start
        self.buckets.zero()
        loss_dict = self.compute_losses(data)
        losses = sum(loss_dict.values())
        self.buckets.begin_backward((self.iter > self.burn_in, self.share_source_pass, self.fuse_consistency,
                                     bool(self.cfg.MODEL.KD_REGULRAZIATION), len(data), tuple(sorted(loss_dict))))
        try:
            losses.backward()
        except BaseException:
            from . import layers
            layers._TOUCH_HOOK[0] = None
            raise
        self.buckets.all_reduce_mean()
        self.optimizer.iteration = self.iter
        self.optimizer.step()
        if self.metrics_period and self.iter % self.metrics_period == 0:
            self._write_metrics(loss_dict, data_time)
        self.iter += 1
        return loss_dict

    def _write_metrics(self, loss_dict, data_time):
        keys = sorted(loss_dict.keys())
        vec = torch.stack([loss_dict[k].detach().float() for k in keys])
        if get_world_size() > 1:
            dist.all_reduce(vec)
            vec = vec / get_world_size()
        vals = vec.cpu().tolist()
        metrics = dict(zip(keys, vals))
        total = sum(vals)
        if not all(map(lambda v: v == v and abs(v) != float("inf"), [total])):
            raise FloatingPointError(f"Loss became infinite or NaN at iteration={self.iter}!\nloss_dict = {metrics}")
        from . import layers
        nf = layers.FP8_SCALES.nonfinite
        if nf is not None and bool(nf.item()):
            raise FloatingPointError(f"An activation or gradient quantised to e4m3 held Inf / NaN at or before iteration={self.iter} (loss_dict = {metrics})")
        if any(bool(f.item()) for f in layers.RPN_SPARSE_OVERFLOW.flags()):
            raise RuntimeError("The RPN head's sparse backward pass found more rows with a gradient than the sampled anchors' count at or "
                               f"before iteration={self.iter}: gradient rows were dropped, and every optimizer step since the previous metrics "
                               "write may have used such a gradient -- the weights are not to be trusted.  Rerun with CDDMSL_RPN_SPARSE_BWD=0")
        self.storage.update(metrics)
        self.storage["total_loss"] = total
        self.storage["data_time"] = data_time


class SyntheticPairedLoader:

    def __init__(self, per_rank_batch, height=800, width=1333, rank=0, device="cuda", num_classes=20, pool=2):
        from . import synthetic
        from .structures import Boxes, Instances
        self.batches = []
        for it in range(pool):
            b = synthetic.make_batch(per_rank_batch, height, width, rank, it, num_classes=num_classes)
            for x in b:
                x["image"], x["image_trgt"] = x["image"].to(device), x["image_trgt"].to(device)
                i = x["instances"]
                x["instances"] = Instances((height, width), gt_boxes=Boxes(i["gt_boxes"].to(device)), gt_classes=i["gt_classes"].to(device))
            self.batches.append(b)
        self.i = 0

    def __iter__(self):
        return self

    def __next__(self):
        b = self.batches[self.i % len(self.batches)]
        self.i += 1
        return b


def limit_host_threads(n=4):
    if torch.get_num_threads() > n:
        torch.set_num_threads(n)


def build_trainer(cfg, per_rank_batch, height=800, width=1333, seed=1):
    from .modeling import build_model
    limit_host_threads()
    rank, _ = get_rank(), get_world_size()
    model = build_model(cfg)
    model.proposal_generator.sample_generator.manual_seed(seed + rank)
    model.roi_heads.sample_generator.manual_seed(seed + rank + 7919)
    model.region_generator.manual_seed(seed + rank + 104729)
    opt = build_optimizer(cfg, model)
    loader = SyntheticPairedLoader(per_rank_batch, height, width, rank, cfg.MODEL.DEVICE, cfg.MODEL.ROI_HEADS.NUM_CLASSES)
    return SimpleTrainer(model, loader, opt, cfg)
```

### cddmsl_amd/hip.py

```python
import ctypes
import math
import os
from ctypes import c_float, c_int, c_long, c_void_p

import torch

from ._lib import check, lib, lib_rpn_sparse, ptr, require_cuda, stream_ptr

DT = {torch.bfloat16: 0, torch.float32: 1}

_L = lib
_LR = lib_rpn_sparse


class _Profiler:

    def __init__(self):
        self.on = False
        self.only = None
        self.events = []
        self.shapes = []

    def enable(self, only=None):
        self.on, self.only, self.events, self.shapes = True, (set(only) if only else None), [], []

    def begin(self, name=None, plan=None):
        if not self.on:
            return None
        if self.only is not None:
            if name is None and plan is not None:
                L = _L()
                L.cddmsl_plan_only(1)
                try:
                    plan()
                finally:
                    L.cddmsl_plan_only(0)
                name = _CONV_KERNEL.get(L.cddmsl_last_kernel())
            if name not in self.only:
                return None
        e = torch.cuda.Event(enable_timing=True)
        e.record()
        return e

    def end(self, e0, name, flops=0.0, shape=None, nbytes=0.0):
        if e0 is None:
            return
        e1 = torch.cuda.Event(enable_timing=True)
        e1.record()
        self.events.append((name, flops, e0, e1, nbytes))
        if shape is not None:
            self.shapes.append((name, shape, flops, e0, e1, nbytes))

    def by_shape(self):
        torch.cuda.synchronize()
        out = {}
        for name, shape, flops, e0, e1, nbytes in self.shapes:
            d = out.setdefault((name, shape), [0, 0.0, 0.0, 0.0])
            d[0] += 1
            d[1] += e0.elapsed_time(e1)
            d[2] += flops
            d[3] += nbytes
        return out

    def collect(self):
        torch.cuda.synchronize()
        out = {}
        for name, flops, e0, e1, nbytes in self.events:
            d = out.setdefault(name, {"flops": 0.0, "ms": 0.0, "launches": 0, "bytes": 0.0})
            d["flops"] += flops
            d["bytes"] += nbytes
            d["ms"] += e0.elapsed_time(e1)
            d["launches"] += 1
        self.on, self.only, self.events = False, None, []
        return out


PROFILE = _Profiler()
_CONV_KERNEL = {10: "k_conv_fwd256_fp8", 11: "k_conv_fwd2", 1: "k_conv_fwd", 2: "k_conv_fwd_reg", 3: "k_conv_fwd256", 4: "k_conv_wgrad", 5: "k_conv_wgrad_dma", 6: "k_wgrad256", 7: "k_gemm_tn_stream", 8: "k_conv3x3_small", 9: "k_gemm_tn_small", 12: "k_wgrad256_fp8",
                13: "k_bottleneck64"}


def _timed(name):
    def deco(fn):
        def wrapper(*a, **k):
            e0 = PROFILE.begin(name)
            r = fn(*a, **k)
            PROFILE.end(e0, name)
            return r
        wrapper.__name__, wrapper.__doc__ = fn.__name__, fn.__doc__
        return wrapper
    return deco


def _dt(t):
# ... 142 lines not shown
def quantize_fp8(x, scale=None, amax=None):
    require_cuda(x, scale, amax)
    assert x.is_contiguous() and x.dtype in (torch.bfloat16, torch.float32) and x.numel() % 8 == 0
    y = torch.empty(x.shape, device=x.device, dtype=torch.uint8)
    check(_L().cddmsl_quantize_fp8(ptr(x), ptr(y), ptr(scale), ptr(amax), x.numel(), 0 if x.dtype == torch.bfloat16 else 1, stream_ptr()),
          "cddmsl_quantize_fp8")
    return y


def conv_fwd_fp8_ok(M, Cin, Cout, KH, KW, pad):
    min_tiles = int(os.environ.get("CDDMSL_FP8_MIN_TILES", "160"))
    min_k = int(os.environ.get("CDDMSL_FP8_MIN_K", "2048"))
    return Cin % 128 == 0 and Cout % 256 == 0 and KH * KW <= 31 and 2 * pad <= KH - 1 and ((M + 255) // 256) * (Cout // 256) >= min_tiles \
        and KH * KW * Cin >= min_k


def conv_fwd_fp8(x8, w8, scale=None, bias=None, residual=None, relu=False, relu_mask=None, pad=0, out_f32=False, emit8=None):
    require_cuda(x8, w8, scale, bias, residual, relu_mask)
    assert x8.dtype == torch.uint8 and w8.dtype == torch.uint8 and x8.is_contiguous() and w8.is_contiguous()
    N, H, W, Cin = x8.shape
    Cout, KH, KW, Cin2 = w8.shape
    assert Cin == Cin2
    Ho, Wo = H + 2 * pad - KH + 1, W + 2 * pad - KW + 1
    y = torch.empty((N, Ho, Wo, Cout), device=x8.device, dtype=torch.float32 if out_f32 else torch.bfloat16)
    for v in (scale, bias):
        assert v is None or (v.dtype == torch.float32 and v.numel() == Cout and v.is_contiguous())
    for v in (residual, relu_mask):
        assert v is None or (v.dtype == torch.bfloat16 and v.is_contiguous() and v.numel() == y.numel())

    y8 = torch.empty(y.shape, device=x8.device, dtype=torch.uint8) if emit8 is not None else None
    assert emit8 is None or not out_f32

    def launch():
        return _L().cddmsl_conv_fwd_fp8(ptr(x8), ptr(w8), ptr(y), ptr(scale), ptr(bias), ptr(residual), ptr(relu_mask),
                                        N, H, W, Cin, Cout, KH, KW, pad, int(relu), int(out_f32), ptr(y8),
                                        ptr(emit8[0]) if emit8 else c_void_p(0), ptr(emit8[1]) if emit8 else c_void_p(0), stream_ptr())
    e0 = PROFILE.begin(name="k_conv_fwd256_fp8") if PROFILE.on else None
    check(launch(), "cddmsl_conv_fwd_fp8")
    PROFILE.end(e0, "k_conv_fwd256_fp8", 2.0 * N * Ho * Wo * Cout * KH * KW * Cin, (N * Ho * Wo, Cout, KH * KW * Cin, KH, 0, 1),
                nbytes=float(x8.numel() + w8.numel() + y.numel() * y.element_size() + (residual.numel() * 2 if residual is not None else 0)
                             + (relu_mask.numel() * 2 if relu_mask is not None else 0)))
    if y8 is not None:
        y._fp8 = (y8, emit8[0].data_ptr())
    return y


@_timed("fp8_dot_nt")
def fp8_dot_nt(a8, b8, alpha=None):
    require_cuda(a8, b8, alpha)
    R, K = a8.shape
    N = b8.shape[0]
    assert a8.dtype == torch.uint8 and b8.dtype == torch.uint8 and a8.is_contiguous() and b8.is_contiguous() and b8.shape[1] == K
    c = torch.empty((R, N), device=a8.device, dtype=torch.float32)
    check(_L().cddmsl_fp8_dot_nt(ptr(a8), ptr(b8), ptr(c), ptr(alpha), R, N, K, N, stream_ptr()), "cddmsl_fp8_dot_nt")
    return c


def pooled_residual_ok(t):
    return t.numel() * t.element_size() < 2 ** 31 and t.shape[-1] % 8 == 0


def linear_fwd(x, w, scale=None, bias=None, residual=None, relu=False, relu_mask=None, out_f32=False):
    M, K = x.shape
    y = conv_fwd(x.view(1, 1, M, K), w.view(w.shape[0], 1, 1, K), scale, bias,
                 None if residual is None else residual.view(1, 1, M, -1), relu,
                 None if relu_mask is None else relu_mask.view(1, 1, M, -1), out_f32=out_f32)
    return y.view(M, w.shape[0])


_WORKSPACE = {}
WORKSPACE_BYTES = 288 << 20


def ensure_workspace(device):
    key = torch.device(device).index or 0
    if key not in _WORKSPACE:
        ws = torch.empty(WORKSPACE_BYTES, dtype=torch.uint8, device=device)
        check(_L().cddmsl_set_workspace(ptr(ws), ctypes.c_long(ws.numel())), "cddmsl_set_workspace")
        _WORKSPACE[key] = ws
    return _WORKSPACE[key]


def conv_wgrad(x, dy, w_shape, scale=None, stride=1, pad=0, pool=False, out=None):
    require_cuda(x, dy, scale, out)
    Cout, KH, KW, Cin = w_shape
    N, H, W, Cin2 = x.shape
    assert Cin == Cin2 and x.dtype == dy.dtype and x.is_contiguous() and dy.is_contiguous()
    assert dy.shape[-1] == Cout and dy.numel() // Cout == (N * (H // 2) * (W // 2) if pool else
                                                          N * ((H + 2 * pad - KH) // stride + 1) * ((W + 2 * pad - KW) // stride + 1))
    if out is None:
        out = torch.zeros(w_shape, device=x.device, dtype=torch.float32)
    assert out.dtype == torch.float32 and out.is_contiguous() and tuple(out.shape) == tuple(w_shape)
    ensure_workspace(x.device)
    def launch():
        return _L().cddmsl_conv_wgrad(ptr(x), ptr(dy), ptr(out), ptr(scale), N, H, W, Cin, Cout, KH, KW, stride, pad,
                                      int(pool), Cout, _dt(x), stream_ptr())
    e0 = PROFILE.begin(plan=launch) if PROFILE.on else None
    st = launch()
    check(st, "cddmsl_conv_wgrad")
    PROFILE.end(e0, _CONV_KERNEL.get(_L().cddmsl_last_kernel(), "conv_wgrad") if e0 is not None else "conv_wgrad",
                2.0 * (dy.numel() // Cout) * Cout * KH * KW * Cin,
                (dy.numel() // Cout, Cout, KH * KW * Cin, KH, int(pool), stride),
                nbytes=float(_conv_input_pixels(N, H, W, (H // 2) if pool else (H + 2 * pad - KH) // stride + 1,
                                                 (W // 2) if pool else (W + 2 * pad - KW) // stride + 1, KH, KW, stride, bool(pool)) * Cin * x.element_size()
                             + dy.numel() * dy.element_size() + out.numel() * 4))
    return out


def conv_wgrad_fp8_ok(M, Cin, Cout, KH, KW, pad, min_m=None, taps_only=True):
    min_m = int(os.environ.get("CDDMSL_FP8_WGRAD_MIN_M", "300000" if min_m is None else str(min_m)))
    return os.environ.get("CDDMSL_FP8_WGRAD", "1") != "0" and (KH * KW > 1 or not taps_only) and M >= min_m \
        and bool(_L().cddmsl_conv_wgrad_fp8_ok(Cin, Cout, KH, KW, pad, Cout))


def conv_wgrad_fp8(x8, dy8, w_shape, scale, pad=0, out=None):
    require_cuda(x8, dy8, scale, out)
    Cout, KH, KW, Cin = w_shape
    N, H, W, Cin2 = x8.shape
    assert Cin == Cin2 and x8.dtype == torch.uint8 and dy8.dtype == torch.uint8 and x8.is_contiguous() and dy8.is_contiguous()
    assert dy8.shape[-1] == Cout and dy8.numel() // Cout == N * H * W and 2 * pad == KH - 1
    assert scale is not None and scale.dtype == torch.float32 and scale.numel() == Cout and scale.is_contiguous()
    if out is None:
        out = torch.zeros(w_shape, device=x8.device, dtype=torch.float32)
    assert out.dtype == torch.float32 and out.is_contiguous() and tuple(out.shape) == tuple(w_shape)
    ensure_workspace(x8.device)
    def launch():
        return _L().cddmsl_conv_wgrad_fp8(ptr(x8), ptr(dy8), ptr(out), ptr(scale), N, H, W, Cin, Cout, KH, KW, pad, Cout, stream_ptr())
    e0 = PROFILE.begin(name="k_wgrad256_fp8") if PROFILE.on else None
    check(launch(), "cddmsl_conv_wgrad_fp8")
    PROFILE.end(e0, "k_wgrad256_fp8", 2.0 * (N * H * W) * Cout * KH * KW * Cin, (N * H * W, Cout, KH * KW * Cin, KH, 0, 1),
                nbytes=float(x8.numel() + dy8.numel() + out.numel() * 4))
    return out


@_timed("weight_prep")
def weight_prep(w_master, scale, dtype, want_fwd=True, want_dgrad=True):
    require_cuda(w_master, scale)
    assert w_master.dtype == torch.float32 and w_master.is_contiguous() and w_master.dim() == 4
    Cout, KH, KW, Cin = w_master.shape
    wf = torch.empty((Cout, KH, KW, Cin), device=w_master.device, dtype=dtype) if want_fwd else None
    wd = torch.empty((Cin, KH, KW, Cout), device=w_master.device, dtype=dtype) if want_dgrad else None
    st = _L().cddmsl_weight_prep(ptr(w_master), ptr(scale), ptr(wf), ptr(wd), Cout, KH, KW, Cin, DT[dtype], stream_ptr())
    check(st, "cddmsl_weight_prep")
    return wf, wd


@_timed("weight_prep")
def weight_prep_multi(table, count, dtype):
    require_cuda(table)
    assert table.dtype == torch.int64 and table.is_contiguous() and table.shape == (count, 8)
    check(_L().cddmsl_weight_prep_multi(ptr(table), count, DT[dtype], stream_ptr()), "cddmsl_weight_prep_multi")


def _f3(v):
    return (c_float * 3)(*[float(x) for x in v])


def _image_table(images_u8):
    import ctypes
    n = len(images_u8)
    ptrs = (ctypes.c_void_p * n)(*[im.data_ptr() for im in images_u8])
    hs = (ctypes.c_int * n)(*[int(im.shape[1]) for im in images_u8])
    ws = (ctypes.c_int * n)(*[int(im.shape[2]) for im in images_u8])
    return ptrs, hs, ws


@_timed("preprocess")
def preprocess(images_u8, Hp, Wp, mean, std, dtype, Cp=None, div255=True):
    require_cuda(*images_u8)
    Cp = Cp or (8 if dtype == torch.bfloat16 else 4)
    out = torch.empty((len(images_u8), Hp, Wp, Cp), device=images_u8[0].device, dtype=dtype)
    m, s = _f3(mean), _f3(std)
    for im in images_u8:
        assert im.dtype == torch.uint8 and im.dim() == 3 and im.shape[0] == 3 and im.is_contiguous()
    ptrs, hs, ws = _image_table(images_u8)
    check(_L().cddmsl_preprocess_batch(ptrs, hs, ws, len(images_u8), ptr(out), Hp, Wp, Cp, m, s, int(div255), DT[dtype], stream_ptr()),
          "cddmsl_preprocess_batch")
    return out


@_timed("preprocess224")
def preprocess224(images_u8, Hp, Wp, mean, std, dtype, size=224, Cp=None):
    require_cuda(*images_u8)
    Cp = Cp or (8 if dtype == torch.bfloat16 else 4)
    if Wp <= Hp:
        RW, RH = size, int(size * Hp / Wp)
    else:
        RH, RW = size, int(size * Wp / Hp)
    top, left = int(round((RH - size) / 2.0)), int(round((RW - size) / 2.0))
    out = torch.empty((len(images_u8), size, size, Cp), device=images_u8[0].device, dtype=dtype)
    m, s = _f3(mean), _f3(std)
    for im in images_u8:
        assert im.dtype == torch.uint8 and im.dim() == 3 and im.is_contiguous()
    ptrs, hs, ws = _image_table(images_u8)
    check(_L().cddmsl_preprocess224_batch(ptrs, hs, ws, len(images_u8), ptr(out), Hp, Wp, RH, RW, top, left, size, Cp,
                                           m, s, DT[dtype], stream_ptr()), "cddmsl_preprocess224_batch")
    return out


from .resample import resample_table as _resample_table


def tta_view_list(sizes, flip):
    return [(int(nh), int(nw), f) for nh, nw in sizes for f in ((False, True) if flip else (False,))]


@_timed("tta_views")
def tta_views(image_u8, sizes, flip, mean, std, dtype, batch_size=3, div255=True):
    import numpy as np
    require_cuda(image_u8)
    assert image_u8.dtype == torch.uint8 and image_u8.dim() == 3 and image_u8.shape[0] == 3 and image_u8.is_contiguous()
# ... 1359 lines not shown
```

### cddmsl_amd/layers.py

```python
import os
import weakref

import torch

from . import hip

_STEP = [0]


def bump_weight_version():
    _STEP[0] += 1


def weight_version():
    return _STEP[0]


_LOAD_GEN = [0]


def note_weights_loaded(*_):
    _LOAD_GEN[0] += 1
    _STEP[0] += 1


def load_generation():
    return _LOAD_GEN[0]


_TOUCHED = set()


_TOUCH_HOOK = [None]


def _grad_buf(p):
    if p.grad is None:
        p.grad = torch.zeros_like(p, memory_format=torch.preserve_format)
    _TOUCHED.add(id(p))
    if _TOUCH_HOOK[0] is not None:
        _TOUCH_HOOK[0](p)
    return p.grad


def take_touched():
    t = set(_TOUCHED)
    _TOUCHED.clear()
    return t


def _ohwi(w):
    if w.dim() == 2:
        return w.view(w.shape[0], 1, 1, w.shape[1])
    v = w.permute(0, 2, 3, 1)
    assert v.is_contiguous(), "conv weights must be channels_last"
    return v


class PreparedWeight:

    _live = weakref.WeakSet()
    _table = None

    def __init__(self, param, scale=None, frozen=False):
        self.param, self.scale, self.frozen = param, scale, frozen
        self._key = None
        self._wf = self._wd = None
        self._dtype, self._used = None, False
        if not frozen:
            PreparedWeight._live.add(self)

    def _sig(self):
        return (self.param.data_ptr(), 0 if self.scale is None else self.scale.data_ptr(), self._wf.data_ptr(),
                0 if self._wd is None else self._wd.data_ptr())

    @staticmethod
    def _refresh_all(dtype):
        items = [pw for pw in PreparedWeight._live if pw._wf is not None and pw._dtype == dtype and pw._used
                 and pw._key is not None and pw._key[2] == pw.param.data_ptr()]
        if not items:
            return
        sig = tuple(pw._sig() for pw in items)
        if PreparedWeight._table is None or PreparedWeight._table[0] != sig or PreparedWeight._table[2] != dtype:
            rows = []
            for pw in items:
                Cout, KH, KW, Cin = _ohwi(pw.param).shape
                rows.append(list(pw._sig()) + [Cout, KH, KW, Cin])
            from ._lib import to_device_async
            PreparedWeight._table = (sig, to_device_async(torch.tensor(rows, dtype=torch.int64), items[0].param.device), dtype)
        hip.weight_prep_multi(PreparedWeight._table[1], len(items), dtype)
        for pw in items:
            pw._key = (dtype, _STEP[0], pw.param.data_ptr(), pw.param._version)
            pw._used = False

    def get(self, dtype, need_dgrad=True):
        key = (dtype, -1 if self.frozen else _STEP[0], self.param.data_ptr(), self.param._version)
        if key != self._key and not self.frozen and self._wf is not None and self._dtype == dtype:
            PreparedWeight._refresh_all(dtype)
        if key != self._key or (need_dgrad and self._wd is None):
            wf, wd = hip.weight_prep(_ohwi(self.param.detach()), self.scale, dtype, True, need_dgrad)
            self._wf, self._wd, self._key, self._dtype = wf, (wd if need_dgrad else None), key, dtype
        self._used = True
        return self._wf, self._wd


class Fp8Slot:
    __slots__ = ("scale", "deq", "amax", "calibrated")

    def __init__(self, scale, deq, amax):
        self.scale, self.deq, self.amax, self.calibrated = scale, deq, amax, False

    def calibrate(self, t):
        if not self.calibrated:
            amax = t.detach().abs().amax().float().view(1)
            ok = torch.isfinite(amax) & (amax > 0)
            sc = torch.where(ok, hip.FP8_MAX / amax.clamp(1e-30, 3.0e38), torch.ones_like(amax))
            self.scale.copy_(sc)
            self.deq.copy_(1.0 / sc)
            FP8_SCALES.note_nonfinite(~torch.isfinite(amax))
            self.calibrated = True

    def emit(self):
        return (self.scale, self.amax) if self.calibrated else None


# ... 482 lines not shown
        p2, bits = hip.avgpool2_fwd_bits(o2)
    else:
        p2 = hip.avgpool2_fwd(o2) if pool else o2
    if pool and px_given is not None and tuple(px_given.shape) == (x.shape[0], x.shape[1] // 2, x.shape[2] // 2, x.shape[3]):
        px = px_given
    else:
        px = hip.avgpool2_fwd(x) if pool else x
    if bp.pw[3] is not None:
        idn = conv_fwd_auto(px, bp.pw[3], bnd[0], bnd[1], f8)
    else:
        idn = x
    out_shape = (p2.shape[0], p2.shape[1], p2.shape[2], _ohwi(bp.w[2]).shape[0])
    out = conv_fwd_auto(p2, bp.pw[2], s3, b3, f8, emit8=fp8_emit_for(next_pw, out_shape, 0, f8), residual=idn, relu=True, out_spec=out_spec)
    return out, ((o1, o2 if bits is None else bits, p2 if pool else None, px if pool else None,
                  (x8, _fp8_made_for(o1, bp.pw[1]) if f8 else None, o2_8), o2_shape) if save else None)


def _block_backward(gs, x, o1, o2, p2, px, bp, need_dx, mask_x, prev_bp=None, c8=(None, None, None), o2_shape=None):
    T = x.dtype
    (s1, _), (s2, _), (s3, _), bnd = bp.bn
    pool = bp.stride > 1
    f8 = bp.fp8 and T == torch.bfloat16
    w1p, w2p, w3p, wdp = bp.w
    shp = lambda w: _ohwi(w).shape
    gs_slot = fp8_slot_of(bp, "_fp8_gs") if f8 else None
    d2_slot = fp8_slot_of(bp.pw[1], "_fp8_g") if f8 else None
    x8, o1_8, o2_8 = c8
    o2_bits = o2.dtype == torch.int32
    o2_shape = tuple(o2.shape) if o2_shape is None else tuple(o2_shape)
    M2 = o2_shape[0] * o2_shape[1] * o2_shape[2]
    if o2_8 is not None and not pool:
        wgrad_auto(o2, gs, bp.pw[2], s3, 0, _ohwi(_grad_buf(w3p)), f8, o2_8, gs_slot, taps_only=False)
    else:
        hip.conv_wgrad(p2 if pool else o2, gs, shp(w3p), s3, out=_ohwi(_grad_buf(w3p)))
    d1_slot = fp8_slot_of(bp.pw[0], "_fp8_g") if f8 and x8 is not None and _fp8_wgrad1x1_wanted(bp.pw[0], M2, f8) else None
    if pool:
        dp2 = dgrad_auto(gs, bp.pw[2], f8, gs_slot)
        if o2_bits:
            dpre2 = hip.avgpool2_bwd_bits(dp2, o2_shape, o2)
        else:
            dpre2 = hip.avgpool2_bwd(dp2, o2_shape, mask=o2, emit8=d2_slot.emit() if f8 and _fp8_dgrad_wanted(bp.pw[1], o2_shape, 1, f8) else None)
    else:
        e8 = d2_slot.emit() if f8 and _fp8_dgrad_wanted(bp.pw[1], o2_shape, 1, f8) else None
        dpre2 = dgrad_auto(gs, bp.pw[2], f8, gs_slot, emit8=e8, relu_mask=o2)
    dpre1 = dgrad_auto(dpre2, bp.pw[1], f8, d2_slot, pad=1, relu_mask=o1, emit8=d1_slot.emit() if d1_slot is not None else None)
    wgrad_auto(o1, dpre2, bp.pw[1], s2, 1, _ohwi(_grad_buf(w2p)), f8, o1_8, d2_slot)
    if d1_slot is not None:
        wgrad_auto(x, dpre1, bp.pw[0], s1, 0, _ohwi(_grad_buf(w1p)), f8, x8, d1_slot, taps_only=False)
    else:
        hip.conv_wgrad(x, dpre1, shp(w1p), s1, out=_ohwi(_grad_buf(w1p)))
    if wdp is not None:
        hip.conv_wgrad(px if pool else x, gs, shp(wdp), bnd[0], out=_ohwi(_grad_buf(wdp)))
    if not need_dx:
        return None
    pooled = False
    if wdp is not None:
        dxb = dgrad_auto(gs, bp.pw[3], f8, gs_slot)
        if pool:
            pooled = x.shape[1] % 2 == 0 and x.shape[2] % 2 == 0 and hip.pooled_residual_ok(dxb)
            if not pooled:
                dxb = hip.avgpool2_bwd(dxb, tuple(x.shape))
    else:
        dxb = gs
    e8 = None
    if f8 and prev_bp is not None and prev_bp.fp8 and not pooled and _fp8_dgrad_wanted(prev_bp.pw[2], x.shape, 0, True):
        e8 = fp8_slot_of(prev_bp, "_fp8_gs").emit()
    return dgrad_auto(dpre1, bp.pw[0], False, None, emit8=e8, residual=dxb, relu_mask=x if mask_x else None, residual_pooled=pooled)


class ResStageFn(torch.autograd.Function):
    @staticmethod
    def forward(ctx, x, anchor, blocks, out_grad_premasked=False, px0=None, out_spec=None):
        ctx.out_grad_premasked = out_grad_premasked
        saved, o1_8s, o2_shapes = [x], [], []
        cur = x
        for bi, bp in enumerate(blocks):
            cur, mids = _block_forward(cur, bp, True, px0 if bi == 0 else None, blocks[bi + 1].pw[0] if bi + 1 < len(blocks) else None,
                                       out_spec if bi + 1 == len(blocks) else None)
            saved += [mids[0], mids[1], mids[2], mids[3], cur]
            o1_8s += list(mids[4])
            o2_shapes.append(mids[5])
        ctx.blocks, ctx.o2_shapes = blocks, o2_shapes
        ctx.save_for_backward(*saved, *o1_8s)
        return cur

    @staticmethod
    def backward(ctx, g):
        blocks = ctx.blocks
        saved, o1_8s = ctx.saved_tensors[:-3 * len(blocks)], ctx.saved_tensors[-3 * len(blocks):]
        need_dx = ctx.needs_input_grad[0]
        gs = g.contiguous() if ctx.out_grad_premasked else hip.relu_bwd(g.contiguous(), saved[-1])
        for i in range(len(blocks) - 1, -1, -1):
            x, o1, o2, p2, px = saved[5 * i: 5 * i + 5]
            gs = _block_backward(gs, x, o1, o2, p2, px, blocks[i], need_dx or i > 0, mask_x=i > 0, prev_bp=blocks[i - 1] if i > 0 else None,
                                 c8=tuple(o1_8s[3 * i: 3 * i + 3]), o2_shape=ctx.o2_shapes[i])
        return gs, None, None, None, None, None


def _fused_stage_ok(x, blocks, out_spec):
    if os.environ.get("CDDMSL_FUSED_BOTTLENECK", "1") == "0" or out_spec is not None:
        return False
    if not (x.is_cuda and x.dtype == torch.bfloat16 and x.dim() == 4 and x.is_contiguous()):
        return False
    cin = x.shape[3]
    for bi, bp in enumerate(blocks):
        if bp.fp8 or bp.stride != 1 or any(v is None for b in bp.bn[:3] for v in b):
            return False
        if tuple(_ohwi(bp.w[0]).shape) != (64, 1, 1, cin) or tuple(_ohwi(bp.w[1]).shape) != (64, 3, 3, 64) or tuple(_ohwi(bp.w[2]).shape) != (256, 1, 1, 64):
            return False
        if bp.w[3] is not None:
            if bi > 0 or cin != 64 or tuple(_ohwi(bp.w[3]).shape) != (256, 1, 1, 64) or any(v is None for v in bp.bn[3]):
                return False
        elif cin != 256:
            return False
        cin = 256
    return bool(blocks) and bool(hip._L().cddmsl_bottleneck64_ok(x.shape[0], x.shape[1], x.shape[2], 0))


def _fused_stage_forward(x, blocks):
    T = x.dtype
    wf = lambda pw: pw.get(T, need_dgrad=False)[0]
    o1 = conv_fwd_auto(x, blocks[0].pw[0], blocks[0].bn[0][0], blocks[0].bn[0][1], False, relu=True)
    cur = x
    for bi, bp in enumerate(blocks):
        nxt = blocks[bi + 1] if bi + 1 < len(blocks) else None
        kw = dict(x0=cur, wd=wf(bp.pw[3]), bnd=bp.bn[3]) if bp.pw[3] is not None else dict(residual=cur)
        if nxt is not None:
            kw.update(w1n=wf(nxt.pw[0]), bn1n=nxt.bn[0])
        cur, o1 = hip.bottleneck64_fwd(o1, wf(bp.pw[1]), bp.bn[1], wf(bp.pw[2]), bp.bn[2], **kw)
    return cur


def res_stage(x, blocks, frozen, out_grad_premasked=False, out_spec=None):
    px0 = getattr(x, "_pooled2", None)
    if frozen or not torch.is_grad_enabled():
        if _fused_stage_ok(x, blocks, out_spec):
            return _fused_stage_forward(x, blocks)
        cur = x
        for bi, bp in enumerate(blocks):
            cur, _ = _block_forward(cur, bp, False, px0 if bi == 0 else None, blocks[bi + 1].pw[0] if bi + 1 < len(blocks) else None,
                                    out_spec if bi + 1 == len(blocks) else None)
        return cur
    return ResStageFn.apply(x, blocks[0].w[0], blocks, out_grad_premasked, px0, out_spec)


class StackHalvesFn(torch.autograd.Function):

    @staticmethod
    def forward(ctx, a, b, full):
        n = a.shape[0]
        assert a.data_ptr() == full.data_ptr() and b.data_ptr() == full[n:].data_ptr() and full.shape[0] == 2 * n and a.shape == b.shape
        ctx.n = n
        return full.view(full.shape)

    @staticmethod
    def backward(ctx, g):
        return g[:ctx.n], g[ctx.n:], None


def stack_halves(a, b, full):
    return StackHalvesFn.apply(a, b, full)


def res_stage_attnpool(x, blocks, frozen, ap):
    fuse = not frozen and torch.is_grad_enabled()
    y = res_stage(x, blocks, frozen, out_grad_premasked=fuse)
    return AttnPoolFn.apply(y, None if ap.frozen else ap.q_w, ap, fuse)


def roi_downsample_on_map(K, out_size, N, H, W):
    if os.environ.get("CDDMSL_ROI_COMMUTE", "1") == "0":
        return False
    v = os.environ.get("CDDMSL_ROI_COMMUTE_DOWN", "")
    if v in ("0", "1"):
        return v == "1"
    return K * (out_size // 2) ** 2 > N * H * W


def _roi_block0_forward(feat, rois, bp, out_size, scale, sr, extra, next_pw=None, on_map=None, save=False):
    T = feat.dtype
    (s1, b1), (s2, b2), (s3, b3), bnd = bp.bn
    w1, _ = bp.pw[0].get(T, False)
    f8 = bp.fp8
    K, E = rois.shape[0], (0 if extra is None else extra.shape[0])
    N, H, W, _ = feat.shape
    z = hip.conv_fwd(feat, w1)
    o1_shape = (K + E, out_size, out_size, z.shape[-1])
    e8 = fp8_emit_for(bp.pw[1], o1_shape, 1, f8) if E == 0 else None
    o1 = hip.roi_align_forward_affine(z, rois, out_size, out_size, scale, sr, True, s1, b1, relu=True, extra_rows=E, emit8=e8)
    del z
    if on_map is None:
        on_map = roi_downsample_on_map(K, out_size, N, H, W)
    if on_map:
        wd, _ = bp.pw[3].get(T, False)
        zd = hip.conv_fwd(feat, wd)
        idn = hip.roi_align_forward_affine(zd, rois, out_size, out_size, scale, sr, True, bnd[0], bnd[1], pooled_only=True, extra_rows=E)
        del zd
        px = None
        if E:
            px = hip.avgpool2_fwd(extra)
            idn[K:].copy_(hip.conv_fwd(px, wd, bnd[0], bnd[1]))
    else:
        px = hip.roi_align_forward_affine(feat, rois, out_size, out_size, scale, sr, True, pooled_only=True, extra_rows=E)
        idn = None
    if E:
        o1[K:].copy_(hip.conv_fwd(extra, w1, s1, b1, relu=True))
        if idn is None:
            px[K:].copy_(hip.avgpool2_fwd(extra))
    o2 = conv_fwd_auto(o1, bp.pw[1], s2, b2, f8, relu=True, pad=1)
    o2_shape = tuple(o2.shape)
    if save and _pool_bits_wanted(bp, o2):
        p2, o2 = hip.avgpool2_fwd_bits(o2)
    else:
        p2 = hip.avgpool2_fwd(o2)
    if idn is None:
        idn = conv_fwd_auto(px, bp.pw[3], bnd[0], bnd[1], f8)
    out_shape = (p2.shape[0], p2.shape[1], p2.shape[2], _ohwi(bp.w[2]).shape[0])
    out = conv_fwd_auto(p2, bp.pw[2], s3, b3, f8, emit8=fp8_emit_for(next_pw, out_shape, 0, f8), residual=idn, relu=True)
    return o1, o2, p2, px, out, (_fp8_made_for(o1, bp.pw[1]) if f8 else None), o2_shape


class RoIStageFn(torch.autograd.Function):

    @staticmethod
    def forward(ctx, feat, anchor, rois, roi_start, blocks, out_size, scale, sr, out_grad_premasked, extra):
        feat = feat.contiguous()
        nxt = lambda i: blocks[i + 1].pw[0] if i + 1 < len(blocks) else None
        on_map = roi_downsample_on_map(rois.shape[0], out_size, feat.shape[0], feat.shape[1], feat.shape[2])
        o1, o2, p2, px, cur, o1_8, o2_shape = _roi_block0_forward(feat, rois, blocks[0], out_size, scale, sr, extra, nxt(0), on_map, save=True)
        saved, o1_8s, o2_shapes = [feat, rois, roi_start, extra, o1, o2, p2, px, cur], [None, o1_8, None], [o2_shape]
        for bi, bp in enumerate(blocks[1:], start=1):
            cur, mids = _block_forward(cur, bp, True, None, nxt(bi))
            saved += [mids[0], mids[1], mids[2], mids[3], cur]
            o1_8s += list(mids[4])
            o2_shapes.append(mids[5])
        ctx.o2_shapes = o2_shapes
        ctx.blocks, ctx.meta = blocks, (out_size, scale, sr, out_grad_premasked, on_map)
        ctx.save_for_backward(*saved, *o1_8s)
        return cur

    @staticmethod
    def backward(ctx, g):
        blocks = ctx.blocks
        saved, o1_8s = ctx.saved_tensors[:-3 * len(blocks)], ctx.saved_tensors[-3 * len(blocks):]
        out_size, scale, sr, premasked, on_map = ctx.meta
        feat, rois, roi_start, extra = saved[:4]
        st = saved[4:]
        gs = g.contiguous() if premasked else hip.relu_bwd(g.contiguous(), st[-1])
        for i in range(len(blocks) - 1, 0, -1):
            o1, o2, p2, px = st[5 * i: 5 * i + 4]
            gs = _block_backward(gs, st[5 * i - 1], o1, o2, p2, px, blocks[i], True, mask_x=True, prev_bp=blocks[i - 1], c8=tuple(o1_8s[3 * i: 3 * i + 3]),
                                 o2_shape=ctx.o2_shapes[i])
        bp = blocks[0]
        o1, o2, p2, px = st[0:4]
        o2_shape = ctx.o2_shapes[0]
        T = o1.dtype
        (s1, _), (s2, _), (s3, _), bnd = bp.bn
        w1p, w2p, w3p, wdp = bp.w
        shp = lambda w: _ohwi(w).shape
        K, E = rois.shape[0], (0 if extra is None else extra.shape[0])
        f8 = bp.fp8 and T == torch.bfloat16
        gs_slot = fp8_slot_of(bp, "_fp8_gs") if f8 else None
        d2_slot = fp8_slot_of(bp.pw[1], "_fp8_g") if f8 else None
        hip.conv_wgrad(p2, gs, shp(w3p), s3, out=_ohwi(_grad_buf(w3p)))
        if o2.dtype == torch.int32:
            dpre2 = hip.avgpool2_bwd_bits(dgrad_auto(gs, bp.pw[2], f8, gs_slot), o2_shape, o2)
        else:
            e8 = d2_slot.emit() if f8 and _fp8_dgrad_wanted(bp.pw[1], o2_shape, 1, f8) else None
            dpre2 = hip.avgpool2_bwd(dgrad_auto(gs, bp.pw[2], f8, gs_slot), o2_shape, mask=o2, emit8=e8)
        dpre1 = dgrad_auto(dpre2, bp.pw[1], f8, d2_slot, pad=1, relu_mask=o1)
        wgrad_auto(o1, dpre2, bp.pw[1], s2, 1, _ohwi(_grad_buf(w2p)), f8, o1_8s[1], d2_slot)
        N, H, W, C = feat.shape
        _, w1d = bp.pw[0].get(T, True)
        dfeat = dextra = dzd = wdd = None
        if on_map:
            _, wdd = bp.pw[3].get(T, True)
            dzd = hip.roi_align_backward(gs[:K], rois, roi_start, (N, H, W, gs.shape[-1]), scale, sr, True, pooled=True)
            hip.conv_wgrad(feat, dzd, shp(wdp), bnd[0], out=_ohwi(_grad_buf(wdp)))
            if E:
                hip.conv_wgrad(px, gs[K:], shp(wdp), bnd[0], out=_ohwi(_grad_buf(wdp)))
        else:
            hip.conv_wgrad(px, gs, shp(wdp), bnd[0], out=_ohwi(_grad_buf(wdp)))
            dxb = dgrad_auto(gs, bp.pw[3], f8, gs_slot)
        dz = hip.roi_align_backward(dpre1[:K], rois, roi_start, (N, H, W, dpre1.shape[-1]), scale, sr, True)
        hip.conv_wgrad(feat, dz, shp(w1p), s1, out=_ohwi(_grad_buf(w1p)))
        if E:
            hip.conv_wgrad(extra, dpre1[K:], shp(w1p), s1, out=_ohwi(_grad_buf(w1p)))
            if ctx.needs_input_grad[9]:
                dxe = hip.conv_fwd(gs[K:], wdd) if on_map else dxb[K:].contiguous()
                dextra = hip.conv_fwd(dpre1[K:], w1d, residual=hip.avgpool2_bwd(dxe, tuple(extra.shape)))
        if ctx.needs_input_grad[0]:
            r = hip.conv_fwd(dzd, wdd) if on_map else hip.roi_align_backward(dxb[:K], rois, roi_start, (N, H, W, C), scale, sr, True, pooled=True)
            dfeat = hip.conv_fwd(dz, w1d, residual=r)
        return dfeat, None, None, None, None, None, None, None, None, dextra


def roi_stage_supported(blocks):
    bp = blocks[0]
    return bp.stride == 2 and bp.w[3] is not None and tuple(bp.w[0].shape[2:]) == (1, 1) and tuple(bp.w[3].shape[2:]) == (1, 1)


def roi_stage(feat, rois, roi_start, blocks, frozen, out_size, scale, sr, extra=None, out_grad_premasked=False):
    assert rois.dim() == 2 and rois.size(1) == 5 and out_size % 2 == 0
    assert extra is None or tuple(extra.shape[1:]) == (out_size, out_size, feat.shape[3])
    if frozen or not torch.is_grad_enabled():
        nxt = lambda i: blocks[i + 1].pw[0] if i + 1 < len(blocks) else None
        cur = _roi_block0_forward(feat.contiguous(), rois, blocks[0], out_size, scale, sr, extra, nxt(0))[4]
        for bi, bp in enumerate(blocks[1:], start=1):
            cur, _ = _block_forward(cur, bp, False, None, nxt(bi))
        return cur
    return RoIStageFn.apply(feat, blocks[0].w[0], rois, roi_start, blocks, out_size, scale, sr, out_grad_premasked, extra)


def roi_stage_attnpool(feat, rois, roi_start, blocks, frozen, ap, out_size, scale, sr, extra=None):
    fuse = not frozen and torch.is_grad_enabled()
    y = roi_stage(feat, rois, roi_start, blocks, frozen, out_size, scale, sr, extra, out_grad_premasked=fuse)
    return AttnPoolFn.apply(y, None if ap.frozen else ap.q_w, ap, fuse)


class RoIAlignFn(torch.autograd.Function):
    @staticmethod
    def forward(ctx, x, rois, roi_start, out_size, scale, sampling_ratio, aligned, with_pooled=False, extra=None):
        K, E = rois.shape[0], (0 if extra is None else extra.shape[0])
        out = hip.roi_align_forward(x, rois, out_size, out_size, scale, sampling_ratio, aligned, with_pooled=with_pooled, extra_rows=E)
        ctx.save_for_backward(rois, roi_start)
        ctx.meta = (tuple(x.shape), scale, sampling_ratio, aligned, K)
# ... 566 lines not shown
```

Before: 171.6.

## Merge weight-gradient convolutions for shared weights into one segmented wgrad launch

Adds a segmented weight-gradient kernel path that handles up to four (x, dy) pairs with different spatial shapes in a single launch. The segment descriptors are read from kernel arguments. A Python-side queue counts the expected gradient contributions per weight during backward, defers them, and launches them together once all have arrived. The goal is to cut per-launch overhead and the underfilled grids of small wgrad launches, such as the ROI and extra-branch uses of shared bottleneck weights. The cost is more bookkeeping and a risk of deferred or misordered accumulation if the expected counts do not match reality.

```diff
diff --git a/__graft_entry__.py b/__graft_entry__.py
--- a/__graft_entry__.py
+++ b/__graft_entry__.py
@@ -6,7 +6,9 @@
 ROOT = os.path.dirname(os.path.abspath(__file__))
 CSRC = os.path.join(ROOT, "cddmsl_amd", "csrc")
 LIB = os.path.join(ROOT, "cddmsl_amd", "libcddmsl_hip.so")
-SIDE_LIBS = {"rpn_sparse.hip": os.path.join(ROOT, "cddmsl_amd", "libcddmsl_rpn_sparse.so")}
+SIDE_LIBS = {"rpn_sparse.hip": os.path.join(ROOT, "cddmsl_amd", "libcddmsl_rpn_sparse.so"),
+             "wgrad_segments.hip": os.path.join(ROOT, "cddmsl_amd", "libcddmsl_wgrad_segments.so")}
+SIDE_SHARED = {"wgrad_segments.hip": ["conv_wgrad.hip"]}
 OBJDIR = os.path.join(ROOT, "build", "obj")
 HIPCC = os.environ.get("HIPCC", "/opt/rocm/bin/hipcc")
 HIPFLAGS = ["--offload-arch=gfx950", "-O3", "-fPIC", "-std=c++17", "-Wno-unused-result", "-ffp-contract=off"]
@@ -37,7 +39,8 @@
         if p.wait() != 0:
             raise RuntimeError(f"hipcc failed on {s}")
     side = {os.path.join(OBJDIR, name[:-4] + ".o"): lib for name, lib in SIDE_LIBS.items()}
-    for lib, members in [(LIB, [o for o in objs if o not in side])] + [(lib, [o]) for o, lib in side.items()]:
+    shared = {os.path.join(OBJDIR, name[:-4] + ".o"): [os.path.join(OBJDIR, m[:-4] + ".o") for m in ms] for name, ms in SIDE_SHARED.items()}
+    for lib, members in [(LIB, [o for o in objs if o not in side])] + [(lib, [o] + shared.get(o, [])) for o, lib in side.items()]:
         if not os.path.exists(lib) or any(os.path.getmtime(o) > os.path.getmtime(lib) for o in members):
             subprocess.check_call([HIPCC, "--offload-arch=gfx950", "-shared", "-fPIC", *members, "-o", lib])
     omk = os.path.join(ROOT, "oracle", "Makefile")
@@ -50,6 +53,7 @@
 
     _lib.lib()
     _lib.lib_rpn_sparse()
+    _lib.lib_wgrad_segments()
 
 
 def smoke():
diff --git a/cddmsl_amd/_lib.py b/cddmsl_amd/_lib.py
--- a/cddmsl_amd/_lib.py
+++ b/cddmsl_amd/_lib.py
@@ -9,9 +9,12 @@
 HEADER_PATH = os.path.join(os.path.dirname(_HERE), "include", "cddmsl_hip.h")
 RPN_SPARSE_LIB_PATH = os.path.join(_HERE, "libcddmsl_rpn_sparse.so")
 RPN_SPARSE_HEADER_PATH = os.path.join(os.path.dirname(_HERE), "include", "cddmsl_rpn_sparse.h")
+WGRAD_SEGMENTS_LIB_PATH = os.path.join(_HERE, "libcddmsl_wgrad_segments.so")
+WGRAD_SEGMENTS_HEADER_PATH = os.path.join(os.path.dirname(_HERE), "include", "cddmsl_wgrad_segments.h")
 
 _lib = None
 _lib_rpn_sparse = None
+_lib_wgrad_segments = None
 
 
 class HipLibraryError(RuntimeError):
@@ -96,6 +99,13 @@
     return _lib_rpn_sparse
 
 
+def lib_wgrad_segments():
+    global _lib_wgrad_segments
+    if _lib_wgrad_segments is None:
+        _lib_wgrad_segments = _load(WGRAD_SEGMENTS_LIB_PATH, WGRAD_SEGMENTS_HEADER_PATH)
+    return _lib_wgrad_segments
+
+
 def stream_ptr():
     return ctypes.c_void_p(torch._C._cuda_getCurrentRawStream(torch.cuda.current_device()))
 
diff --git a/cddmsl_amd/csrc/conv_wgrad.hip b/cddmsl_amd/csrc/conv_wgrad.hip
--- a/cddmsl_amd/csrc/conv_wgrad.hip
+++ b/cddmsl_amd/csrc/conv_wgrad.hip
@@ -189,8 +189,9 @@
   static constexpr int MSTEP = 8;
 };
 
-template <typename T>
-__global__ __launch_bounds__(256, 2) void k_conv_wgrad_dma(WgradArgs p) {
+template <typename T, typename A = WgradArgs>
+__global__ __launch_bounds__(256, 2) void k_conv_wgrad_dma(A p) {
+  constexpr bool SEG = std::is_same<A, WgradSegArgs>::value;
   constexpr int ES = Mma<T>::ES;
   constexpr int COLS = 256 / ES;
   __shared__ __attribute__((aligned(16))) u32x4 lds[2][2][WM * 16];
@@ -205,7 +206,8 @@
   const int split = bid;
   const int n0 = tile_n * COLS, k0 = tile_k * COLS;
   const int mt0 = split * p.mtiles_per_split;
-  const int total_mt = (p.M + WM - 1) / WM;
+  int total_mt;
+  if constexpr (SEG) total_mt = p.total_mt; else total_mt = (p.M + WM - 1) / WM;
   const int mt1 = min(mt0 + p.mtiles_per_split, total_mt);
 
   const int cc = t & 15, rb = t >> 4;
@@ -251,6 +253,40 @@
 #pragma unroll
     for (int i = 0; i < 4; ++i) { m[i] += WM; pd[i] += dstep; px[i] += xstep; }
   };
+  WgradSeg S = {};
+  int seg_end = 0, mtb = 0, ml0 = 0;
+  const char* pdb = nullptr;
+  const char* pxb = nullptr;
+  auto stage_seg = [&](int buf, int mt) {
+    if constexpr (SEG) {
+      if (mt >= seg_end) {
+        S = wgrad_seg_of(p, mt, &seg_end);
+        mtb = mt;
+        ml0 = (mt - S.mt0) * WM + rb;
+        pdb = S.dy + ((long)ml0 * p.ldd) * ES + (long)nc * 16;
+        pxb = S.x + (((long)ml0 + (long)(ky - p.pad) * S.Wi + (kx - p.pad)) * p.xrs) * 16 + (long)coff * 16;
+      }
+      const int ml = ml0 + (mt - mtb) * WM;
+      const char* db = pdb + (long)(mt - mtb) * dstep;
+      const char* xb = pxb + (long)(mt - mtb) * xstep;
+#pragma unroll
+      for (int i = 0; i < 4; ++i)
+        glds16((ml + 16 * i < S.M && vn) ? db + ((long)(16 * i) * p.ldd) * ES : zp, &lds[buf][0][(4 * wvu + 16 * i) * 16]);
+#pragma unroll
+      for (int i = 0; i < 4; ++i) {
+        const int mi = ml + 16 * i;
+        bool ok = (mi < S.M) & vk;
+        if (taps) {
+          unsigned mm = min((unsigned)mi, (unsigned)(S.M - 1));
+          unsigned tq = fdiv(mm, S.dWo);
+          unsigned ox = mm - tq * S.Wi;
+          unsigned oy = tq - fdiv(tq, S.dHo) * S.Hi;
+          ok = ok & ((unsigned)((int)oy - p.pad + ky) < (unsigned)S.Hi) & ((unsigned)((int)ox - p.pad + kx) < (unsigned)S.Wi);
+        }
+        glds16(ok ? xb + ((long)(16 * i) * p.xrs) * 16 : zp, &lds[buf][1][(4 * wvu + 16 * i) * 16]);
+      }
+    }
+  };
 
   constexpr int WT = COLS / 2;
   constexpr int NT = WT / 32;
@@ -270,11 +306,11 @@
     offb[i] = TrFragS<T>::prep(wk * WT + i * 32, lane);
   }
 
-  if (mt0 < mt1) stage(0);
+  if (mt0 < mt1) { if constexpr (SEG) stage_seg(0, mt0); else stage(0); }
   for (int mt = mt0; mt < mt1; ++mt) {
     const int cur = (mt - mt0) & 1;
     if (mt + 1 < mt1) {
-      stage(cur ^ 1);
+      if constexpr (SEG) stage_seg(cur ^ 1, mt + 1); else stage(cur ^ 1);
       asm volatile("s_waitcnt vmcnt(8)" ::: "memory");
     } else {
       asm volatile("s_waitcnt vmcnt(0)" ::: "memory");
@@ -626,7 +662,9 @@
   }
 }
 
-__global__ __launch_bounds__(512) void k_wgrad256(WgradArgs p) {
+template <typename A = WgradArgs>
+__global__ __launch_bounds__(512) void k_wgrad256(A p) {
+  constexpr bool SEG = std::is_same<A, WgradSegArgs>::value;
   __shared__ __attribute__((aligned(16))) u32x4 lds[2 * 2 * 2 * 64 * 16];
   const int t = threadIdx.x, lane = t & 63;
 #ifdef CDDMSL_TILE_STAMPS
@@ -643,7 +681,9 @@
   const int tile_n = bid % ntn; bid /= ntn;
   const int n0 = tile_n * 256, k0 = tile_k * 256;
   const int mt0 = bid * p.mtiles_per_split;
-  const int nmt = min(p.mtiles_per_split, (p.M + WM - 1) / WM - mt0);
+  int total_mt;
+  if constexpr (SEG) total_mt = p.total_mt; else total_mt = (p.M + WM - 1) / WM;
+  const int nmt = min(p.mtiles_per_split, total_mt - mt0);
   const bool taps = !(p.KH == 1 && p.KW == 1);
 
   const int rb = t >> 4, cl = (t & 15) ^ fsw(rb);
@@ -664,9 +704,39 @@
   const int mrow = mt0 * WM + rb;
 
   char* const L = (char*)lds;
+  WgradSeg S = {};
+  int seg_end = 0, Tb = 0, Mrem = 0;
+  int mrow_s = 0;
+  __amdgpu_buffer_rsrc_t rds = rd, rxs = rx;
+  unsigned vxs[2] = {0u, 0u};
+  auto seek = [&](int T) {
+    if constexpr (SEG) {
+      if (mt0 + T >= seg_end) {
+        S = wgrad_seg_of(p, mt0 + T, &seg_end);
+        Tb = T;
+        const int ml = (mt0 + T - S.mt0) * WM;
+        Mrem = S.M - ml;
+        mrow_s = ml + rb;
+        rds = __builtin_amdgcn_make_buffer_rsrc((void*)(S.dy + ((long)ml * p.ldd + n0) * 2), 0, 0x80000000u, 0x00020000);
+        rxs = __builtin_amdgcn_make_buffer_rsrc((void*)(S.x + ((long)ml - p.pad * S.Wi - p.pad) * p.xrs * 16), 0, 0x80000000u, 0x00020000);
+#pragma unroll
+        for (int i = 0; i < 2; ++i) vxs[i] = (unsigned)((((i * 32 + rb) + ky * S.Wi + kx) * p.xrs + coff) * 16);
+      }
+    }
+  };
   auto stageD = [&](auto H, int buf, int T) {
     constexpr int h = decltype(H)::value;
     char* dst = L + (buf << 16) + (h << 14) + wvu * 1024;
+    if constexpr (SEG) {
+      seek(T);
+#pragma unroll
+      for (int i = 0; i < 2; ++i) {
+        const unsigned inv = (rb + (T - Tb) * WM + i * 32 < Mrem) ? 0u : 0x80000000u;
+        __builtin_amdgcn_raw_ptr_buffer_load_lds(rds, (__attribute__((address_space(3))) void*)(dst + i * 8192 - h * 128), 16,
+                                                 (int)(vd[i] | inv), (int)((T - Tb) * dstep), h * 128, 0);
+      }
+      return;
+    }
 #pragma unroll
     for (int i = 0; i < 2; ++i) {
       const unsigned inv = (mrow + T * WM + i * 32 < p.M) ? 0u : 0x80000000u;
@@ -676,6 +746,23 @@
   };
   unsigned xinv[2];
   auto validX = [&](int T) {
+    if constexpr (SEG) {
+      seek(T);
+#pragma unroll
+      for (int i = 0; i < 2; ++i) {
+        const int m = mrow_s + (T - Tb) * WM + i * 32;
+        bool ok = m < S.M;
+        if (taps) {
+          const unsigned mm = min((unsigned)m, (unsigned)(S.M - 1));
+          const unsigned tq = fdiv(mm, S.dWo);
+          const unsigned ox = mm - tq * S.Wi;
+          const unsigned oy = tq - fdiv(tq, S.dHo) * S.Hi;
+          ok = ok & ((unsigned)((int)oy - p.pad + ky) < (unsigned)S.Hi) & ((unsigned)((int)ox - p.pad + kx) < (unsigned)S.Wi);
+        }
+        xinv[i] = ok ? 0u : 0x80000000u;
+      }
+      return;
+    }
 #pragma unroll
     for (int i = 0; i < 2; ++i) {
       const int m = mrow + T * WM + i * 32;
@@ -693,6 +780,13 @@
   auto stageX = [&](auto J, int buf, int T) {
     constexpr int j = decltype(J)::value;
     char* dst = L + (buf << 16) + (1 << 15) + (j << 14) + wvu * 1024;
+    if constexpr (SEG) {
+#pragma unroll
+      for (int i = 0; i < 2; ++i)
+        __builtin_amdgcn_raw_ptr_buffer_load_lds(rxs, (__attribute__((address_space(3))) void*)(dst + i * 8192 - j * 64), 16,
+                                                 (int)(vxs[i] | xinv[i]), (int)((T - Tb) * xstep), j * 64, 0);
+      return;
+    }
 #pragma unroll
     for (int i = 0; i < 2; ++i)
       __builtin_amdgcn_raw_ptr_buffer_load_lds(rx, (__attribute__((address_space(3))) void*)(dst + i * 8192 - j * 64), 16,
@@ -1060,8 +1154,8 @@
   return ws != nullptr && blocks * tile_floats * 4 <= ws_bytes;
 }
 
-template <int WAVES, int FR>
-static void launch_wgrad_split(void (*kernel)(WgradArgs), WgradArgs& a, const Plan& p, hipStream_t st, void* wsp, long ws_bytes) {
+template <int WAVES, int FR, typename A>
+static void launch_wgrad_split(void (*kernel)(A), A& a, const Plan& p, hipStream_t st, void* wsp, long ws_bytes) {
   constexpr int TN = WAVES == 8 ? 256 : 128, SLOTS = WAVES * FR * 64;
   const int ntn = (a.Cout + TN - 1) / TN, ntk = (a.K + TN - 1) / TN;
   const bool ws = p.splits > 1 && use_workspace((long)p.gx, SLOTS * 4, wsp, ws_bytes);
@@ -1074,7 +1168,7 @@
 void launch_wgrad(WgradArgs& a, const Plan& p, Operand op, hipStream_t st, void* ws, long ws_bytes) {
   switch (p.kernel) {
     case 12: launch_wgrad_split<8, 32>(k_wgrad256_f8, a, p, st, ws, ws_bytes); break;
-    case 6: launch_wgrad_split<8, 32>(k_wgrad256, a, p, st, ws, ws_bytes); break;
+    case 6: launch_wgrad_split<8, 32>(k_wgrad256<WgradArgs>, a, p, st, ws, ws_bytes); break;
     case 5:
       if (op == OP_BF16) launch_wgrad_split<4, 16>(k_conv_wgrad_dma<__bf16>, a, p, st, ws, ws_bytes);
       else hipLaunchKernelGGL(k_conv_wgrad_dma<float>, dim3(p.gx), dim3(256), 0, st, a);
@@ -1083,6 +1177,11 @@
       if (op == OP_BF16) hipLaunchKernelGGL(k_conv_wgrad<__bf16>, dim3(p.gx), dim3(256), 0, st, a);
       else hipLaunchKernelGGL(k_conv_wgrad<float>, dim3(p.gx), dim3(256), 0, st, a);
   }
+}
+
+void launch_wgrad_segments(WgradSegArgs& a, const Plan& p, hipStream_t st, void* ws, long ws_bytes) {
+  if (p.kernel == 6) launch_wgrad_split<8, 32>(k_wgrad256<WgradSegArgs>, a, p, st, ws, ws_bytes);
+  else launch_wgrad_split<4, 16>(k_conv_wgrad_dma<__bf16, WgradSegArgs>, a, p, st, ws, ws_bytes);
 }
 
 void launch_gemm_tn(const WgradArgs& p, Operand op, const Plan& pl, int batch, int mode, hipStream_t st) {
diff --git a/cddmsl_amd/csrc/gemm_common.h b/cddmsl_amd/csrc/gemm_common.h
--- a/cddmsl_amd/csrc/gemm_common.h
+++ b/cddmsl_amd/csrc/gemm_common.h
@@ -137,6 +137,34 @@
 };
 
 constexpr int WM = 64;
+
+constexpr int WSEG_MAX = 4;
+struct WgradSeg {
+  const char* x;
+  const char* dy;
+  int M, Hi, Wi, mt0;
+  FastDiv dWo, dHo;
+};
+struct WgradSegArgs : WgradArgs {
+  int total_mt;
+  WgradSeg seg[WSEG_MAX];
+};
+__device__ __forceinline__ WgradSeg wgrad_seg_of(const WgradSegArgs& p, int mt, int* end) {
+  const int e1 = p.seg[1].mt0, e2 = p.seg[2].mt0, e3 = p.seg[3].mt0;
+  const int s = (mt >= e1) + (mt >= e2) + (mt >= e3);
+  *end = s == 0 ? e1 : s == 1 ? e2 : s == 2 ? e3 : 0x7fffffff;
+  typedef const __attribute__((address_space(4))) char* kchar;
+  typedef const __attribute__((address_space(4))) int* kint;
+  static_assert(sizeof(WgradSeg) % 4 == 0, "WgradSeg is read as dwords");
+#pragma clang diagnostic push
+#pragma clang diagnostic ignored "-Winvalid-offsetof"
+  const kint q = (kint)((kchar)__builtin_amdgcn_kernarg_segment_ptr() + __builtin_offsetof(WgradSegArgs, seg)) + s * (int)(sizeof(WgradSeg) / 4);
+#pragma clang diagnostic pop
+  union { WgradSeg seg; int w[sizeof(WgradSeg) / 4]; } u;
+#pragma unroll
+  for (int i = 0; i < (int)(sizeof(WgradSeg) / 4); ++i) u.w[i] = q[i];
+  return u.seg;
+}
 constexpr int WROW = 16 + 4;
 
 __device__ __forceinline__ int fsw(int row) { return ((row & 3) << 2) | ((row >> 2) & 3); }
@@ -186,6 +214,7 @@
 __attribute__((visibility("hidden"))) void launch_fwd_tile128(const ConvArgs& a, const Plan& p, Operand op, hipStream_t st);
 __attribute__((visibility("hidden"))) void launch_fwd_tile256(const ConvArgs& a, const Plan& p, Operand op, hipStream_t st, void* ws, long ws_bytes);
 __attribute__((visibility("hidden"))) void launch_wgrad(WgradArgs& a, const Plan& p, Operand op, hipStream_t st, void* ws, long ws_bytes);
+__attribute__((visibility("hidden"))) void launch_wgrad_segments(WgradSegArgs& a, const Plan& p, hipStream_t st, void* ws, long ws_bytes);
 __attribute__((visibility("hidden"))) void launch_gemm_tn(const WgradArgs& p, Operand op, const Plan& pl, int batch, int mode, hipStream_t st);
 __attribute__((visibility("hidden"))) void launch_attnpool_dx(const WgradArgs& p, unsigned gx, unsigned gy, int nbatch, int bpb, hipStream_t st);
 __attribute__((visibility("hidden"))) bool record_kernel(int id);
diff --git a/cddmsl_amd/csrc/gemm_conv.hip b/cddmsl_amd/csrc/gemm_conv.hip
--- a/cddmsl_amd/csrc/gemm_conv.hip
+++ b/cddmsl_amd/csrc/gemm_conv.hip
@@ -1,4 +1,5 @@
 #include "gemm_common.h"
+#include "wgrad_host.h"
 
 namespace {
 
@@ -225,89 +226,6 @@
                       relu, out_f32, y8, q8, amax8, stream);
 }
 
-static bool wgrad256_ok(const WgradArgs& a, int batch) {
-  const long mode = env_int("CDDMSL_GEMM256", 1);
-  if (mode == 0) return false;
-  if ((a.Cout & 255) || (a.K & 255) || (a.cpp & 7) || (a.ldd & 7)) return false;
-  if (mode == 2) return true;
-  return (long)(a.Cout / 256) * (a.K / 256) * batch * ((a.M + WM - 1) / WM) >= env_int("CDDMSL_WGRAD256_MIN", 4000);
-}
-static bool wgrad256_span_ok(int mtiles_per_split, int Wi, long row_bytes) {
-  return ((long)mtiles_per_split * WM + WM + 2L * Wi + 2) * row_bytes + (1L << 20) < (1L << 31);
-}
-
-static int even_split(int total_mt, long* splits) {
-  const int mps = (int)((total_mt + *splits - 1) / *splits);
-  *splits = (total_mt + mps - 1) / mps;
-  return mps;
-}
-
-static long split_512_rounds(long tiles, int total_mt, bool taps) {
-  bool forced;
-  const long target = env_int("CDDMSL_WGRAD_BLOCKS", taps ? 1024 : 512, &forced);
-  const long maxs = (total_mt + 7) / 8;
-  long splits = 1;
-  const long r0 = (target + 511) / 512;
-  double best = -1.0;
-  for (long r = r0; r <= r0 + 1; ++r) {
-    long c = (512 * r) / tiles;
-    if (c < 1) c = 1;
-    if (c > maxs) c = maxs;
-    long real = c;
-    even_split(total_mt, &real);
-    const long blocks = tiles * real, rounds = (blocks + 511) / 512;
-    const double eff = (double)blocks / (512.0 * rounds);
-    if (eff > best + 0.03) { best = eff; splits = c; }
-    if (c == maxs) break;
-  }
-  if (forced) { splits = (target + tiles - 1) / tiles; if (splits > maxs) splits = maxs; }
-  return splits < 1 ? 1 : splits;
-}
-
-static long split_256_rounds(long tiles, int total_mt) {
-  const long maxs = (total_mt + 15) / 16;
-  long sp = 1;
-  double best = -1.0;
-  for (int r = 1; r <= 6; ++r) {
-    long c = (256L * r) / tiles;
-    if (c < 1) continue;
-    if (c > maxs) c = maxs;
-    const long blocks = tiles * c, rounds = (blocks + 255) / 256;
-    const double eff = (double)blocks / (256.0 * rounds);
-    if (eff > best + 0.02) { best = eff; sp = c; }
-    if (c == maxs) break;
-  }
-  return sp;
-}
-
-static Plan plan_wgrad(const WgradArgs& a, Operand op, int batch) {
-  const int es = elem_size(op), total_mt = (a.M + WM - 1) / WM;
-  const long tiles256 = (long)(a.Cout / 256) * (a.K / 256);
-  const long row_bytes = (long)a.ldd * es > a.xrs * 16L ? (long)a.ldd * es : a.xrs * 16L;
-  if (op == OP_FP8) {
-    long sp = split_256_rounds(tiles256, total_mt);
-    const int mps = even_split(total_mt, &sp);
-    if (!wgrad256_span_ok(mps, a.Wi, row_bytes)) return {};
-    return {12, (unsigned)(tiles256 * sp), 1, (int)sp, mps};
-  }
-  const int cols = 256 / es;
-  const long tiles = (long)((a.Cout + cols - 1) / cols) * ((a.K + cols - 1) / cols);
-  long splits = split_512_rounds(tiles, total_mt, !(a.KH == 1 && a.KW == 1));
-  const int mps = even_split(total_mt, &splits);
-  if (tiles * splits > 0x7fffffffL) return {};
-  const bool same = !a.pool && a.stride == 1 && a.Ho == a.Hi && a.Wo == a.Wi;
-  if (same && op == OP_BF16 && wgrad256_ok(a, batch)) {
-    bool forced;
-    const long want = env_int("CDDMSL_WGRAD256_BLOCKS", 0, &forced);
-    const long maxs = (total_mt + 15) / 16;
-    long sp = forced ? (want + tiles256 - 1) / tiles256 : split_256_rounds(tiles256, total_mt);
-    if (sp > maxs) sp = maxs;
-    if (sp < 1) sp = 1;
-    const int mps256 = even_split(total_mt, &sp);
-    if (wgrad256_span_ok(mps256, a.Wi, row_bytes)) return {6, (unsigned)(tiles256 * sp), 1, (int)sp, mps256};
-  }
-  return {same ? 5 : 4, (unsigned)(tiles * splits), 1, (int)splits, mps};
-}
 
 extern "C" int cddmsl_set_workspace(void* ptr, long bytes) {
   if (bytes < 0 || (ptr == nullptr && bytes != 0) || ((size_t)ptr & 15)) return CDDMSL_ERR_ARG;
@@ -326,26 +244,11 @@
 
 static int fill_wgrad(WgradArgs& a, Operand op, const void* x, const void* dy, float* dw, const float* scale, int Nimg, int Hi,
                       int Wi, int Cin, int Cout, int KH, int KW, int stride, int pad, int pool, int ldd) {
-  const int es = elem_size(op);
-  if (Nimg < 0 || Hi <= 0 || Wi <= 0 || Cin <= 0 || Cout <= 0 || KH <= 0 || KW <= 0 || stride <= 0) return CDDMSL_ERR_ARG;
-  if ((Cin * es) % 16 != 0 || (Cout * es) % 16 != 0 || (ldd * es) % 16 != 0) return CDDMSL_ERR_ARG;
-  if (pool && (KH != 1 || KW != 1 || pad != 0 || stride != 1)) return CDDMSL_ERR_ARG;
-  a.x = (const char*)x; a.dy = (const char*)dy; a.dw = dw; a.scale = scale;
-  a.Nimg = Nimg; a.Hi = Hi; a.Wi = Wi; a.Cin = Cin; a.Cout = Cout; a.KH = KH; a.KW = KW; a.stride = stride; a.pad = pad;
-  a.ldd = ldd; a.pool = pool;
-  if (pool) { a.Ho = Hi / 2; a.Wo = Wi / 2; }
-  else { a.Ho = (Hi + 2 * pad - KH) / stride + 1; a.Wo = (Wi + 2 * pad - KW) / stride + 1; }
-  if (a.Ho <= 0 || a.Wo <= 0) return CDDMSL_ERR_ARG;
-  long M = (long)Nimg * a.Ho * a.Wo;
-  if (M > 0x7fffff00L) return CDDMSL_ERR_ARG;
-  a.M = (int)M; a.cpp = Cin * es / 16; a.Kc = KH * KW * a.cpp; a.K = KH * KW * Cin; a.ncc = Cout * es / 16;
-  a.mtiles_per_split = 0;
-  a.dWo = make_fastdiv((unsigned)a.Wo); a.dHo = make_fastdiv((unsigned)a.Ho);
-  a.xrs = a.cpp; a.ldo = a.K; a.direct = 0; a.bx = a.bd = a.bo = 0;
+  const int st = fill_wgrad_args(a, op, x, dy, dw, scale, Nimg, Hi, Wi, Cin, Cout, KH, KW, stride, pad, pool, ldd);
 #ifdef CDDMSL_TILE_STAMPS
   a.tstamps = g_tile_stamps;
 #endif
-  return CDDMSL_OK;
+  return st;
 }
 
 extern "C" int cddmsl_conv_wgrad(const void* x, const void* dy, float* dw, const float* scale, int Nimg, int Hi,
diff --git a/cddmsl_amd/csrc/wgrad_host.h b/cddmsl_amd/csrc/wgrad_host.h
--- /dev/null
+++ b/cddmsl_amd/csrc/wgrad_host.h
@@ -0,0 +1,111 @@
+#pragma once
+#include "gemm_common.h"
+
+namespace {
+
+static bool wgrad256_ok(const WgradArgs& a, int batch) {
+  const long mode = env_int("CDDMSL_GEMM256", 1);
+  if (mode == 0) return false;
+  if ((a.Cout & 255) || (a.K & 255) || (a.cpp & 7) || (a.ldd & 7)) return false;
+  if (mode == 2) return true;
+  return (long)(a.Cout / 256) * (a.K / 256) * batch * ((a.M + WM - 1) / WM) >= env_int("CDDMSL_WGRAD256_MIN", 4000);
+}
+static bool wgrad256_span_ok(int mtiles_per_split, int Wi, long row_bytes) {
+  return ((long)mtiles_per_split * WM + WM + 2L * Wi + 2) * row_bytes + (1L << 20) < (1L << 31);
+}
+
+static int even_split(int total_mt, long* splits) {
+  const int mps = (int)((total_mt + *splits - 1) / *splits);
+  *splits = (total_mt + mps - 1) / mps;
+  return mps;
+}
+
+static long split_512_rounds(long tiles, int total_mt, bool taps) {
+  bool forced;
+  const long target = env_int("CDDMSL_WGRAD_BLOCKS", taps ? 1024 : 512, &forced);
+  const long maxs = (total_mt + 7) / 8;
+  long splits = 1;
+  const long r0 = (target + 511) / 512;
+  double best = -1.0;
+  for (long r = r0; r <= r0 + 1; ++r) {
+    long c = (512 * r) / tiles;
+    if (c < 1) c = 1;
+    if (c > maxs) c = maxs;
+    long real = c;
+    even_split(total_mt, &real);
+    const long blocks = tiles * real, rounds = (blocks + 511) / 512;
+    const double eff = (double)blocks / (512.0 * rounds);
+    if (eff > best + 0.03) { best = eff; splits = c; }
+    if (c == maxs) break;
+  }
+  if (forced) { splits = (target + tiles - 1) / tiles; if (splits > maxs) splits = maxs; }
+  return splits < 1 ? 1 : splits;
+}
+
+static long split_256_rounds(long tiles, int total_mt) {
+  const long maxs = (total_mt + 15) / 16;
+  long sp = 1;
+  double best = -1.0;
+  for (int r = 1; r <= 6; ++r) {
+    long c = (256L * r) / tiles;
+    if (c < 1) continue;
+    if (c > maxs) c = maxs;
+    const long blocks = tiles * c, rounds = (blocks + 255) / 256;
+    const double eff = (double)blocks / (256.0 * rounds);
+    if (eff > best + 0.02) { best = eff; sp = c; }
+    if (c == maxs) break;
+  }
+  return sp;
+}
+
+static Plan plan_wgrad(const WgradArgs& a, Operand op, int batch) {
+  const int es = elem_size(op), total_mt = (a.M + WM - 1) / WM;
+  const long tiles256 = (long)(a.Cout / 256) * (a.K / 256);
+  const long row_bytes = (long)a.ldd * es > a.xrs * 16L ? (long)a.ldd * es : a.xrs * 16L;
+  if (op == OP_FP8) {
+    long sp = split_256_rounds(tiles256, total_mt);
+    const int mps = even_split(total_mt, &sp);
+    if (!wgrad256_span_ok(mps, a.Wi, row_bytes)) return {};
+    return {12, (unsigned)(tiles256 * sp), 1, (int)sp, mps};
+  }
+  const int cols = 256 / es;
+  const long tiles = (long)((a.Cout + cols - 1) / cols) * ((a.K + cols - 1) / cols);
+  long splits = split_512_rounds(tiles, total_mt, !(a.KH == 1 && a.KW == 1));
+  const int mps = even_split(total_mt, &splits);
+  if (tiles * splits > 0x7fffffffL) return {};
+  const bool same = !a.pool && a.stride == 1 && a.Ho == a.Hi && a.Wo == a.Wi;
+  if (same && op == OP_BF16 && wgrad256_ok(a, batch)) {
+    bool forced;
+    const long want = env_int("CDDMSL_WGRAD256_BLOCKS", 0, &forced);
+    const long maxs = (total_mt + 15) / 16;
+    long sp = forced ? (want + tiles256 - 1) / tiles256 : split_256_rounds(tiles256, total_mt);
+    if (sp > maxs) sp = maxs;
+    if (sp < 1) sp = 1;
+    const int mps256 = even_split(total_mt, &sp);
+    if (wgrad256_span_ok(mps256, a.Wi, row_bytes)) return {6, (unsigned)(tiles256 * sp), 1, (int)sp, mps256};
+  }
+  return {same ? 5 : 4, (unsigned)(tiles * splits), 1, (int)splits, mps};
+}
+
+static int fill_wgrad_args(WgradArgs& a, Operand op, const void* x, const void* dy, float* dw, const float* scale, int Nimg, int Hi,
+                      int Wi, int Cin, int Cout, int KH, int KW, int stride, int pad, int pool, int ldd) {
+  const int es = elem_size(op);
+  if (Nimg < 0 || Hi <= 0 || Wi <= 0 || Cin <= 0 || Cout <= 0 || KH <= 0 || KW <= 0 || stride <= 0) return CDDMSL_ERR_ARG;
+  if ((Cin * es) % 16 != 0 || (Cout * es) % 16 != 0 || (ldd * es) % 16 != 0) return CDDMSL_ERR_ARG;
+  if (pool && (KH != 1 || KW != 1 || pad != 0 || stride != 1)) return CDDMSL_ERR_ARG;
+  a.x = (const char*)x; a.dy = (const char*)dy; a.dw = dw; a.scale = scale;
+  a.Nimg = Nimg; a.Hi = Hi; a.Wi = Wi; a.Cin = Cin; a.Cout = Cout; a.KH = KH; a.KW = KW; a.stride = stride; a.pad = pad;
+  a.ldd = ldd; a.pool = pool;
+  if (pool) { a.Ho = Hi / 2; a.Wo = Wi / 2; }
+  else { a.Ho = (Hi + 2 * pad - KH) / stride + 1; a.Wo = (Wi + 2 * pad - KW) / stride + 1; }
+  if (a.Ho <= 0 || a.Wo <= 0) return CDDMSL_ERR_ARG;
+  long M = (long)Nimg * a.Ho * a.Wo;
+  if (M > 0x7fffff00L) return CDDMSL_ERR_ARG;
+  a.M = (int)M; a.cpp = Cin * es / 16; a.Kc = KH * KW * a.cpp; a.K = KH * KW * Cin; a.ncc = Cout * es / 16;
+  a.mtiles_per_split = 0;
+  a.dWo = make_fastdiv((unsigned)a.Wo); a.dHo = make_fastdiv((unsigned)a.Ho);
+  a.xrs = a.cpp; a.ldo = a.K; a.direct = 0; a.bx = a.bd = a.bo = 0;
+  return CDDMSL_OK;
+}
+
+}
diff --git a/cddmsl_amd/csrc/wgrad_segments.hip b/cddmsl_amd/csrc/wgrad_segments.hip
--- /dev/null
+++ b/cddmsl_amd/csrc/wgrad_segments.hip
@@ -0,0 +1,60 @@
+#include "wgrad_host.h"
+#include "cddmsl_wgrad_segments.h"
+#include <climits>
+
+static_assert(CDDMSL_WGRAD_MAX_SEGMENTS == WSEG_MAX, "header and kernels disagree on the number of segments");
+
+extern "C" int cddmsl_conv_wgrad_segments(const cddmsl_wgrad_segment* segs, int nseg, float* dw, const float* scale, int Cin, int Cout,
+                                          int KH, int KW, int stride, int pad, int pool, int ldd, int dtype, void* ws, long ws_bytes,
+                                          int plan_only, int* kernel, void* stream) {
+  if (kernel) *kernel = 0;
+  if (segs == nullptr || nseg < 1 || nseg > WSEG_MAX || dtype != 0) return CDDMSL_ERR_ARG;
+  if (stride != 1 || pool != 0 || KH != KW || 2 * pad != KH - 1) return CDDMSL_ERR_ARG;
+  if (ws_bytes < 0 || (ws == nullptr && ws_bytes != 0) || ((size_t)ws & 15)) return CDDMSL_ERR_ARG;
+  for (int i = 0; i < nseg; ++i) {
+    const cddmsl_wgrad_segment& s = segs[i];
+    if (s.Cin != Cin || s.Cout != Cout || s.KH != KH || s.KW != KW || s.dtype != 0) return CDDMSL_ERR_ARG;
+    if (s.x == nullptr || s.dy == nullptr) return CDDMSL_ERR_ARG;
+  }
+  WgradSegArgs a;
+  int st = fill_wgrad_args(a, OP_BF16, segs[0].x, segs[0].dy, dw, scale, segs[0].Nimg, segs[0].Hi, segs[0].Wi, Cin, Cout, KH, KW, 1, pad, 0, ldd);
+  if (st != CDDMSL_OK) return st;
+  if (nseg == 1) {
+    if (a.M == 0) return CDDMSL_OK;
+    WgradArgs& one = a;
+    const Plan p = plan_wgrad(one, OP_BF16, 1);
+    if (p.kernel == 0) return CDDMSL_ERR_ARG;
+    if (kernel) *kernel = p.kernel;
+    if (plan_only) return CDDMSL_OK;
+    one.mtiles_per_split = p.mtiles_per_split;
+    launch_wgrad(one, p, OP_BF16, (hipStream_t)stream, ws, ws_bytes);
+    return launch_status();
+  }
+  long total_mt = 0;
+  int n = 0, wmax = 0;
+  for (int i = 0; i < nseg; ++i) {
+    WgradArgs g;
+    st = fill_wgrad_args(g, OP_BF16, segs[i].x, segs[i].dy, dw, scale, segs[i].Nimg, segs[i].Hi, segs[i].Wi, Cin, Cout, KH, KW, 1, pad, 0, ldd);
+    if (st != CDDMSL_OK) return st;
+    if (g.M == 0) continue;
+    WgradSeg& s = a.seg[n++];
+    s.x = g.x; s.dy = g.dy; s.M = g.M; s.Hi = g.Hi; s.Wi = g.Wi; s.mt0 = (int)total_mt; s.dWo = g.dWo; s.dHo = g.dHo;
+    total_mt += (g.M + WM - 1) / WM;
+    if (g.Wi > wmax) wmax = g.Wi;
+  }
+  if (n == 0) return CDDMSL_OK;
+  if (total_mt * WM > 0x7fffff00L) return CDDMSL_ERR_ARG;
+  for (int i = n; i < WSEG_MAX; ++i) { a.seg[i] = a.seg[0]; a.seg[i].mt0 = INT_MAX; }
+  a.total_mt = (int)total_mt;
+  a.x = a.dy = nullptr;
+  a.Nimg = 1; a.Hi = a.Ho = 1; a.Wi = a.Wo = wmax; a.M = (int)(total_mt * WM);
+  a.dWo = make_fastdiv((unsigned)wmax); a.dHo = make_fastdiv(1u);
+  const WgradArgs& whole = a;
+  Plan p = plan_wgrad(whole, OP_BF16, 1);
+  if (p.kernel != 5 && p.kernel != 6) return CDDMSL_ERR_ARG;
+  if (kernel) *kernel = p.kernel;
+  if (plan_only) return CDDMSL_OK;
+  a.mtiles_per_split = p.mtiles_per_split;
+  launch_wgrad_segments(a, p, (hipStream_t)stream, ws, ws_bytes);
+  return launch_status();
+}
diff --git a/cddmsl_amd/engine.py b/cddmsl_amd/engine.py
--- a/cddmsl_amd/engine.py
+++ b/cddmsl_amd/engine.py
@@ -227,16 +227,19 @@
         data = next(self._data_loader_iter)
         data_time = time.perf_counter() - start
         self.buckets.zero()
-        loss_dict = self.compute_losses(data)
-        losses = sum(loss_dict.values())
-        self.buckets.begin_backward((self.iter > self.burn_in, self.share_source_pass, self.fuse_consistency,
-                                     bool(self.cfg.MODEL.KD_REGULRAZIATION), len(data), tuple(sorted(loss_dict))))
-        try:
-            losses.backward()
-        except BaseException:
-            from . import layers
-            layers._TOUCH_HOOK[0] = None
-            raise
+        from . import hip
+        with hip.wgrad_merging() as merged:
+            loss_dict = self.compute_losses(data)
+            losses = sum(loss_dict.values())
+            self.buckets.begin_backward((self.iter > self.burn_in, self.share_source_pass, self.fuse_consistency,
+                                         bool(self.cfg.MODEL.KD_REGULRAZIATION), len(data), tuple(sorted(loss_dict))))
+            try:
+                losses.backward()
+            except BaseException:
+                from . import layers
+                layers._TOUCH_HOOK[0] = None
+                raise
+            assert not hip.WGRAD_QUEUE.pending, "a weight gradient was still held back after backward(): an announced use never arrived"
         self.buckets.all_reduce_mean()
         self.optimizer.iteration = self.iter
         self.optimizer.step()
diff --git a/cddmsl_amd/hip.py b/cddmsl_amd/hip.py
--- a/cddmsl_amd/hip.py
+++ b/cddmsl_amd/hip.py
@@ -5,11 +5,12 @@
 
 import torch
 
-from ._lib import check, lib, lib_rpn_sparse, ptr, require_cuda, stream_ptr
+from ._lib import check, lib, lib_rpn_sparse, lib_wgrad_segments, ptr, require_cuda, stream_ptr
 
 DT = {torch.bfloat16: 0, torch.float32: 1}
 
 _L = lib
+_LW = lib_wgrad_segments
 _LR = lib_rpn_sparse
 
 
@@ -318,6 +319,12 @@
 
 
 def conv_wgrad(x, dy, w_shape, scale=None, stride=1, pad=0, pool=False, out=None):
+    if out is not None and WGRAD_QUEUE.expected and WGRAD_QUEUE.arrive(x, dy, tuple(w_shape), scale, stride, pad, pool, out):
+        return out
+    return _conv_wgrad_now(x, dy, w_shape, scale, stride, pad, pool, out)
+
+
+def _conv_wgrad_now(x, dy, w_shape, scale=None, stride=1, pad=0, pool=False, out=None):
     require_cuda(x, dy, scale, out)
     Cout, KH, KW, Cin = w_shape
     N, H, W, Cin2 = x.shape
@@ -343,6 +350,168 @@
     return out
 
 
+class WgradSegment(ctypes.Structure):
+    _fields_ = [("x", ctypes.c_void_p), ("dy", ctypes.c_void_p), ("Nimg", ctypes.c_int), ("Hi", ctypes.c_int), ("Wi", ctypes.c_int),
+                ("Cin", ctypes.c_int), ("Cout", ctypes.c_int), ("KH", ctypes.c_int), ("KW", ctypes.c_int), ("dtype", ctypes.c_int)]
+
+
+_SEG_DTYPE = {torch.bfloat16: 0, torch.float32: 1, torch.uint8: 2}
+
+
+def wgrad_segment_array(segs, KH, KW):
+    arr = (WgradSegment * len(segs))()
+    for a, (x, dy) in zip(arr, segs):
+        assert x.dim() == 4 and x.is_contiguous() and dy.is_contiguous()
+        a.x, a.dy = x.data_ptr(), dy.data_ptr()
+        a.Nimg, a.Hi, a.Wi, a.Cin, a.Cout = x.shape[0], x.shape[1], x.shape[2], x.shape[3], dy.shape[-1]
+        a.KH, a.KW, a.dtype = KH, KW, _SEG_DTYPE.get(x.dtype, 3) if x.dtype == dy.dtype else 3
+    return arr
+
+
+def conv_wgrad_segments_plan(segs, w_shape, pad=0):
+    Cout, KH, KW, Cin = w_shape
+    k = ctypes.c_int(0)
+    arr = wgrad_segment_array(segs, KH, KW)
+    check(_LW().cddmsl_conv_wgrad_segments(arr, len(segs), None, None, Cin, Cout, KH, KW, 1, pad, 0, Cout, 0, None, 0, 1, ctypes.byref(k), None),
+          "cddmsl_conv_wgrad_segments (plan)")
+    return k.value
+
+
+def conv_wgrad_segments(segs, w_shape, scale=None, pad=0, out=None):
+    Cout, KH, KW, Cin = w_shape
+    for x, dy in segs:
+        require_cuda(x, dy)
+        assert dy.numel() // dy.shape[-1] == x.shape[0] * x.shape[1] * x.shape[2]
+    require_cuda(scale, out)
+    dev = segs[0][0].device
+    if out is None:
+        out = torch.zeros(w_shape, device=dev, dtype=torch.float32)
+    assert out.dtype == torch.float32 and out.is_contiguous() and tuple(out.shape) == tuple(w_shape)
+    ws = ensure_workspace(dev)
+    arr = wgrad_segment_array(segs, KH, KW)
+    k = ctypes.c_int(0)
+    e0 = PROFILE.begin(name=_CONV_KERNEL.get(conv_wgrad_segments_plan(segs, w_shape, pad)) if PROFILE.only is not None else None) if PROFILE.on else None
+    st = _LW().cddmsl_conv_wgrad_segments(arr, len(segs), ptr(out), ptr(scale), Cin, Cout, KH, KW, 1, pad, 0, Cout, 0, ptr(ws),
+                                          ctypes.c_long(ws.numel()), 0, ctypes.byref(k), stream_ptr())
+    check(st, "cddmsl_conv_wgrad_segments")
+    M = sum(dy.numel() // Cout for _, dy in segs)
+    PROFILE.end(e0, _CONV_KERNEL.get(k.value, "conv_wgrad"), 2.0 * M * Cout * KH * KW * Cin, (M, Cout, KH * KW * Cin, KH, 0, 1),
+                nbytes=float(sum(x.numel() * x.element_size() + dy.numel() * dy.element_size() for x, dy in segs) + out.numel() * 4))
+    return out
+
+
+def wgrad_merge_enabled():
+    return os.environ.get("CDDMSL_WGRAD_MERGE", "1") != "0"
+
+
+WGRAD_MERGE_MAX_MACS = 1 << 37
+
+
+def wgrad_merge_max_macs():
+    return int(os.environ.get("CDDMSL_WGRAD_MERGE_MACS", WGRAD_MERGE_MAX_MACS))
+
+
+class WgradQueue:
+
+    def __init__(self):
+        self.expected = {}
+        self.pending = {}
+        self.depth = 0
+        self.step = 0
+        self.launch_one = _conv_wgrad_now
+        self.launch_many = conv_wgrad_segments
+
+    def expect(self, buf, uses=1):
+        if not (self.depth and uses > 0 and wgrad_merge_enabled()):
+            return False
+        k = buf.data_ptr()
+        self.expected[k] = self.expected.get(k, 0) + uses
+        return True
+
+    def withdraw(self, buf, uses, step):
+        key = buf.data_ptr()
+        left = self.expected.get(key)
+        if step != self.step or left is None:
+            return
+        if left > uses:
+            self.expected[key] = left - uses
+        else:
+            del self.expected[key]
+            self._launch(key)
+
+    def _launch(self, key):
+        ent = self.pending.pop(key, None)
+        if ent is None:
+            return
+        (w_shape, pad, _), out, scale, segs = ent
+        macs = sum(dy.numel() for _, dy in segs) * w_shape[1] * w_shape[2] * w_shape[3]
+        if len(segs) == 1 or macs > wgrad_merge_max_macs():
+            for x, dy in segs:
+                self.launch_one(x, dy, w_shape, scale, 1, pad, False, out)
+        else:
+            self.launch_many(segs, w_shape, scale, pad, out)
+
+    def arrive(self, x, dy, w_shape, scale, stride, pad, pool, out):
+        key = out.data_ptr()
+        left = self.expected.get(key)
+        if left is None:
+            return False
+        Cout, KH, KW, Cin = w_shape
+        meta = (w_shape, pad, None if scale is None else scale.data_ptr())
+        covered = (wgrad_merge_enabled() and x.dtype == torch.bfloat16 and dy.dtype == torch.bfloat16 and stride == 1 and not pool
+                   and KH == KW and 2 * pad == KH - 1 and x.dim() == 4 and x.shape[3] == Cin and x.is_contiguous() and dy.is_contiguous()
+                   and dy.shape[-1] == Cout and dy.numel() // Cout == x.shape[0] * x.shape[1] * x.shape[2]
+                   and dy.numel() * KH * KW * Cin <= wgrad_merge_max_macs())
+        ent = self.pending.get(key)
+        if covered and ent is not None and (ent[0] != meta or len(ent[3]) >= 4):
+            covered = False
+        if covered:
+            if ent is None:
+                ent = self.pending[key] = (meta, out, scale, [])
+            ent[3].append((x, dy))
+        self._count(key, left)
+        return covered
+
+    def _count(self, key, left):
+        if left > 1:
+            self.expected[key] = left - 1
+        else:
+            del self.expected[key]
+            self._launch(key)
+
+    def arrive_elsewhere(self, out):
+        left = self.expected.get(out.data_ptr()) if self.expected else None
+        if left is not None:
+            self._count(out.data_ptr(), left)
+
+    def flush(self):
+        n = len(self.pending)
+        for key in list(self.pending):
+            self._launch(key)
+        self.expected.clear()
+        self.step += 1
+        return n
+
+
+WGRAD_QUEUE = WgradQueue()
+
+
+class wgrad_merging:
+
+    def __enter__(self):
+        if WGRAD_QUEUE.depth == 0:
+            WGRAD_QUEUE.flush()
+        WGRAD_QUEUE.depth += 1
+        self.left = 0
+        return self
+
+    def __exit__(self, *exc):
+        WGRAD_QUEUE.depth -= 1
+        if WGRAD_QUEUE.depth == 0:
+            self.left = WGRAD_QUEUE.flush()
+        return False
+
+
 def conv_wgrad_fp8_ok(M, Cin, Cout, KH, KW, pad, min_m=None, taps_only=True):
     min_m = int(os.environ.get("CDDMSL_FP8_WGRAD_MIN_M", "300000" if min_m is None else str(min_m)))
     return os.environ.get("CDDMSL_FP8_WGRAD", "1") != "0" and (KH * KW > 1 or not taps_only) and M >= min_m \
@@ -363,6 +532,7 @@
     def launch():
         return _L().cddmsl_conv_wgrad_fp8(ptr(x8), ptr(dy8), ptr(out), ptr(scale), N, H, W, Cin, Cout, KH, KW, pad, Cout, stream_ptr())
     e0 = PROFILE.begin(name="k_wgrad256_fp8") if PROFILE.on else None
+    WGRAD_QUEUE.arrive_elsewhere(out)
     check(launch(), "cddmsl_conv_wgrad_fp8")
     PROFILE.end(e0, "k_wgrad256_fp8", 2.0 * (N * H * W) * Cout * KH * KW * Cin, (N * H * W, Cout, KH * KW * Cin, KH, 0, 1),
                 nbytes=float(x8.numel() + dy8.numel() + out.numel() * 4))
diff --git a/cddmsl_amd/layers.py b/cddmsl_amd/layers.py
--- a/cddmsl_amd/layers.py
+++ b/cddmsl_amd/layers.py
@@ -41,6 +41,32 @@
     if _TOUCH_HOOK[0] is not None:
         _TOUCH_HOOK[0](p)
     return p.grad
+
+
+class _WgradUses:
+
+    def __init__(self):
+        self.step = hip.WGRAD_QUEUE.step if hip.WGRAD_QUEUE.depth else None
+        self.uses = []
+
+    def expect(self, w, uses=1):
+        if self.step is None or w is None or uses <= 0:
+            return
+        if w.grad is None:
+            w.grad = torch.zeros_like(w, memory_format=torch.preserve_format)
+        if hip.WGRAD_QUEUE.expect(w.grad, uses):
+            self.uses.append((w.grad, uses))
+
+    def expect_block(self, bp):
+        for w in bp.w:
+            self.expect(w)
+
+    def ran(self):
+        self.uses = []
+
+    def __del__(self):
+        for buf, uses in self.uses:
+            hip.WGRAD_QUEUE.withdraw(buf, uses, self.step)
 
 
 def take_touched():
@@ -689,11 +715,15 @@
             o2_shapes.append(mids[5])
         ctx.blocks, ctx.o2_shapes = blocks, o2_shapes
         ctx.save_for_backward(*saved, *o1_8s)
+        ctx.wgrad_uses = _WgradUses()
+        for bp in blocks:
+            ctx.wgrad_uses.expect_block(bp)
         return cur
 
     @staticmethod
     def backward(ctx, g):
         blocks = ctx.blocks
+        ctx.wgrad_uses.ran()
         saved, o1_8s = ctx.saved_tensors[:-3 * len(blocks)], ctx.saved_tensors[-3 * len(blocks):]
         need_dx = ctx.needs_input_grad[0]
         gs = g.contiguous() if ctx.out_grad_premasked else hip.relu_bwd(g.contiguous(), saved[-1])
@@ -844,11 +874,21 @@
         ctx.o2_shapes = o2_shapes
         ctx.blocks, ctx.meta = blocks, (out_size, scale, sr, out_grad_premasked, on_map)
         ctx.save_for_backward(*saved, *o1_8s)
+        E = 0 if extra is None or extra.shape[0] == 0 else 1
+        w1p, w2p, w3p, wdp = blocks[0].w
+        u = ctx.wgrad_uses = _WgradUses()
+        u.expect(w1p, 1 + E)
+        u.expect(w2p)
+        u.expect(w3p)
+        u.expect(wdp, 1 + E if on_map else 1)
+        for bp in blocks[1:]:
+            u.expect_block(bp)
         return cur
 
     @staticmethod
     def backward(ctx, g):
         blocks = ctx.blocks
+        ctx.wgrad_uses.ran()
         saved, o1_8s = ctx.saved_tensors[:-3 * len(blocks)], ctx.saved_tensors[-3 * len(blocks):]
         out_size, scale, sr, premasked, on_map = ctx.meta
         feat, rois, roi_start, extra = saved[:4]
diff --git a/include/cddmsl_wgrad_segments.h b/include/cddmsl_wgrad_segments.h
--- /dev/null
+++ b/include/cddmsl_wgrad_segments.h
@@ -0,0 +1,24 @@
+#ifndef CDDMSL_WGRAD_SEGMENTS_H
+#define CDDMSL_WGRAD_SEGMENTS_H
+
+#ifdef __cplusplus
+extern "C" {
+#endif
+
+#define CDDMSL_WGRAD_MAX_SEGMENTS 4
+
+typedef struct cddmsl_wgrad_segment {
+  const void* x;
+  const void* dy;
+  int Nimg, Hi, Wi;
+  int Cin, Cout, KH, KW, dtype;
+} cddmsl_wgrad_segment;
+
+int cddmsl_conv_wgrad_segments(const cddmsl_wgrad_segment* segs, int nseg, float* dw, const float* scale, int Cin, int Cout,
+                               int KH, int KW, int stride, int pad, int pool, int ldd, int dtype, void* ws, long ws_bytes,
+                               int plan_only, int* kernel, void* stream);
+
+#ifdef __cplusplus
+}
+#endif
+#endif
```

After: 172.9 (median of 6 runs). About the same (+0.8%).
